# HaploConduct/HaploConduct

Hardware: AMD Instinct MI355X
Metric: candidate overlaps scored/sec (edge-calc scoring pass: compute_overlap + overlap_score + admission class, candidates resident in HBM; the whole stage from the overlaps text: stage_end_to_end) (higher is better)
Workload: dtype f64; 1 GPU; c3: 500000 synthetic 2x150 bp read pairs, 6 quality values (SURVEY 8(d)), 100000000 p-p candidates per GPU; read_pairs=500000, genome_len=90000, quality_alphabet=6, candidates_per_gpu=100000000, record_bytes=16, parallelism=candidate shards x1, replicated read store

## Files before the change

haploconduct_amd/csrc/hc_kernels.hip:

```cpp
#include <hip/hip_runtime.h>
#include <stdint.h>
#include <stdlib.h>

#include <algorithm>
#include <cstdio>
#include <string>

#include "../../include/hcedge.h"
#include "hc_device.h"
#include "hc_resolve.h"
#include "hc_ctx.h"

#ifndef HC_ABLATE
#define HC_ABLATE 0
#endif

namespace hc {

template <typename SymT, bool WIDE>
__global__ __launch_bounds__(256) void encode_store_kernel(const uint8_t* __restrict__ bases,
                                                           const uint8_t* __restrict__ quals,
                                                           const uint64_t* __restrict__ raw_off,
                                                           const uint64_t* __restrict__ seq_off,
                                                           const uint32_t* __restrict__ rc_delta,
                                                           const uint8_t* __restrict__ qmap,
                                                           uint32_t n_seq, uint32_t K, SymT* __restrict__ sym,
                                                           uint8_t* __restrict__ seq_bad, uint32_t slot_align) {
    const uint32_t lane = threadIdx.x & 63;
    const uint32_t wave = (blockIdx.x * blockDim.x + threadIdx.x) >> 6;
    const uint32_t n_waves = (gridDim.x * blockDim.x) >> 6;
    const bool dup = sizeof(SymT) == 1 && !WIDE && lut_lg(K) == 3;
    const SymT nsym = WIDE ? (SymT)(kWideN << 2) : (SymT)((K << 3) | kCodeN | (dup ? (K & 3u) << 6 : 0u));
    for (uint32_t q = wave; q < n_seq; q += n_waves) {
        const uint64_t r0 = raw_off[q];
        const uint32_t len = (uint32_t)(raw_off[q + 1] - r0);
        const uint64_t f0 = seq_off[q];
        const uint64_t stride = slot_stride(len, sizeof(SymT), slot_align);
        const uint64_t rc0 = f0 + rc_delta[q];
        uint32_t bad = 0;
        for (uint32_t i = lane; i < (uint32_t)stride; i += 64) {
            if (i < len) {
                const uint8_t b = bases[r0 + i];
                const uint8_t qi = qmap[quals[r0 + i]];
                uint32_t code;
                switch (b) {
                    case 'A': code = 0; break;
                    case 'C': code = 1; break;
                    case 'G': code = 2; break;
                    case 'T': code = 3; break;
                    case 'N': code = kCodeN; break;
                    default: code = kCodeBadBase; bad = 1; break;
                }
                uint32_t qx = qi;
                if (WIDE) {
                    uint32_t b2 = code < 4 ? code : 0u;
                    if (code == kCodeN) qx = kWideN;
                    if (code == kCodeBadBase) qx = kWideBadBase;
                    if (qi == 255) { qx = kWideBadQual; b2 = 0; }
                    const uint32_t rb2 = qx >= wide_first(lut_lg(K)) ? 3u - b2 : 0u;
                    sym[f0 + i] = (SymT)((qx << 2) | b2);
                    sym[rc0 + (len - 1 - i)] = (SymT)((qx << 2) | rb2);
                } else {
                    if (code == kCodeN) qx = K;
                    if (code == kCodeBadBase) qx = K + 1;
                    if (qi == 255) {
                        code = kCodeBadQual;
                        qx = K + 1;
                    }
                    const uint32_t rcode = code < 4 ? 3 - code : code;
                    const uint32_t qbits = (qx << 3) | (dup ? (qx & 3u) << 6 : 0u);
                    sym[f0 + i] = (SymT)(qbits | code);
                    sym[rc0 + (len - 1 - i)] = (SymT)(qbits | rcode);
                }
            } else {
                sym[f0 + i] = nsym;
                sym[rc0 + i] = nsym;
            }
        }
        const unsigned long long any_bad = __ballot(bad != 0);
        if (lane == 0) seq_bad[q] = any_bad ? 1 : 0;
    }
}

__global__ __launch_bounds__(256) void build_read_desc_kernel(const uint32_t* __restrict__ read_first_seq,
                                                              const uint64_t* __restrict__ seq_off,
                                                              const uint64_t* __restrict__ raw_off,
                                                              const uint8_t* __restrict__ seq_bad, const uint32_t* __restrict__ rc_delta,
                                                              uint32_t n_reads, ReadDesc* __restrict__ out) {
    const uint32_t r = blockIdx.x * blockDim.x + threadIdx.x;
    if (r >= n_reads) return;
    const uint32_t f = read_first_seq[r];
    const bool paired = (read_first_seq[r + 1] - f) == 2;
    ReadDesc d;
    d.off1 = seq_off[f];
    d.len1 = (uint32_t)(raw_off[f + 1] - raw_off[f]);
    d.flags = (paired ? kReadPaired : 0u) | (seq_bad[f] ? kReadBadBase1 : 0u);
    d.off2 = 0;
    d.len2 = 0;
    if (paired) {
        d.off2 = seq_off[f + 1];
        d.len2 = (uint32_t)(raw_off[f + 2] - raw_off[f + 1]);
        d.flags |= seq_bad[f + 1] ? kReadBadBase2 : 0u;
    }
    d.rc_delta = rc_delta[f];
    out[r] = d;
}

struct SubScore {
    double x;
    uint32_t mm, n;
    uint32_t err;
};

template <typename SymT>
struct Tr;
template <>
struct Tr<uint8_t> {
    static constexpr int kSymsPerWord = 4;
    static constexpr int kWords = 4;
    static constexpr uint32_t kLow1 = 0x01010101u;
    static constexpr int kSymBits = 8;
};
template <>
struct Tr<uint16_t> {
    static constexpr int kSymsPerWord = 2;
    static constexpr int kWords = 8;
    static constexpr uint32_t kLow1 = 0x00010001u;
    static constexpr int kSymBits = 16;
};

typedef const __attribute__((address_space(3))) double lds_cdouble;
__device__ __forceinline__ double lds_f64(uint32_t byte_addr) {
#if HC_ABLATE & 1
    return __hiloint2double(0x3C000000 | (int)(byte_addr & 0xFFFFu), (int)byte_addr);
#else
    return *(lds_cdouble*)(uintptr_t)byte_addr;
#endif
}

template <typename SymT>
__device__ __noinline__ SubScore score_sub_slow(const SymT* __restrict__ a, const SymT* __restrict__ b, uint32_t L, uint32_t Kp) {
    const uint32_t lg = lut_lg(Kp - 2u);
    SubScore r;
    r.x = -__builtin_inf();
    r.mm = 1;
    r.n = 1;
    r.err = 0;
    const bool wide = sizeof(SymT) == 1 && lg >= 6;
    auto kind = [&](uint32_t sy) -> uint32_t {
        if (wide) {
            const uint32_t q = sy >> 2;
            return q == kWideN ? 1u : (q == kWideBadQual ? 2u : (q == kWideBadBase ? 3u : 0u));
        }
        const uint32_t c = sy & 7u;
        return c == kCodeN ? 1u : (c == kCodeBadQual ? 2u : (c == kCodeBadBase ? 3u : 0u));
    };
    for (uint32_t i = 0; i < L; ++i)
        if (kind(a[i]) == 2u || kind(b[i]) == 2u) {
            r.err = 1;
            return r;
        }
    double S = 0.0;
    uint32_t cn = 0, cm = 0;
    for (uint32_t i = 0; i < L; ++i) {
        const uint32_t sa = a[i], sb = b[i];
        const uint32_t ka = kind(sa), kb = kind(sb);
        if (ka == 3u || kb == 3u) {
            r.err = 1;
            return r;
        }
        if (ka == 1u || kb == 1u) continue;
        const uint32_t m = wide ? ((sa & 3u) != (sb & 3u)) : ((sa & 7u) != (sb & 7u));
        const uint32_t qmask = sizeof(SymT) == 1 ? (1u << lg) - 1u : 0xFFFFu;
        const uint32_t qa = wide ? sa >> 2 : (sa >> 3) & qmask, qb = wide ? sb >> 2 : (sb >> 3) & qmask;
        const uint32_t addr = sizeof(SymT) == 1 ? lut_addr_u8(lg, qa, qb, m) : lut_addr_u16(Kp, qa, qb, m);
        const double t = lds_f64(addr);
        if (t == __builtin_inf()) return r;
        S += t;
        cn += 1;
        cm += m;
    }
    if (cn == 0) return r;
    r.x = (1.0 / (double)cn) * S;
    r.mm = cm;
    r.n = cn;
    return r;
}

template <typename SymT, int LG>
__device__ __forceinline__ void half_chunk_terms(const uint32_t* wa, const uint32_t* wb, uint32_t Kp, double (&t)[8], uint32_t& cn4,
                                                 uint32_t& cm4) {
    using T = Tr<SymT>;
#pragma unroll
    for (int jj = 0; jj < T::kWords / 2; ++jj) {
        const uint32_t aw = wa[jj];
        const uint32_t bw = wb[jj];
        const uint32_t e = aw ^ bw;
        if (sizeof(SymT) == 1 && LG >= 6) {
            constexpr uint32_t k80 = 0x80808080u;
            uint32_t ua = (aw << 1) | aw, ub = (bw << 1) | bw;
            if (LG == 7) {
                ua |= ua << 2;
                ub |= ub << 2;
            }
            const uint32_t nm = __builtin_amdgcn_bitop3_b32(ua, k80, ub, 0x4C);
            const uint32_t mk = __builtin_amdgcn_bitop3_b32((e << 7) | (e << 6), k80, nm, 0x40);
            asm("v_bcnt_u32_b32 %0, %1, %0" : "+v"(cn4) : "v"(nm));
            asm("v_bcnt_u32_b32 %0, %1, %0" : "+v"(cm4) : "v"(mk));
            const uint32_t lo = __builtin_amdgcn_bitop3_b32(e << 1, 0xF8F8F8F8u, aw, 0x48);
            const uint32_t z = __builtin_amdgcn_bitop3_b32(e >> 7, 0x01010101u, mk, 0xEA);
            const uint32_t hi = __builtin_amdgcn_bitop3_b32(aw >> 1, 0x7E7E7E7Eu, z, 0xE2);
#pragma unroll
            for (int k = 0; k < 4; ++k)
                t[jj * 4 + k] = lds_f64(__builtin_amdgcn_perm(hi, lo, 0x0C0C0000u | ((4u + k) << 8) | (uint32_t)k));
            continue;
        }
        constexpr uint32_t kFlag = T::kLow1 << 2;
        const uint32_t nm = __builtin_amdgcn_bitop3_b32(aw, kFlag, bw, 0xC8);
        const uint32_t mk = __builtin_amdgcn_bitop3_b32((e << 1) | (e << 2), kFlag, nm, 0x40);
        cn4 += nm;
        cm4 += mk;
        if (sizeof(SymT) == 1) {
            uint32_t lo, hi;
            if (LG == 5) {
                lo = e & 0xF8F8F8F8u;
                hi = ((aw >> 3) & 0x1F1F1F1Fu) | (mk << 3);
            } else if (LG == 4) {
                lo = (e & 0x78787878u) | ((aw << 4) & 0x80808080u);
                hi = ((aw >> 4) & 0x07070707u) | (mk << 1);
            } else {
                lo = (e & 0x38383838u) | (aw & 0xC0C0C0C0u);
                hi = (aw & 0x38383838u) | mk;
            }
#pragma unroll
            for (int k = 0; k < 4; ++k)
                t[jj * 4 + k] = lds_f64(__builtin_amdgcn_perm(hi, lo, 0x0C0C0000u | ((4u + k) << 8) | (uint32_t)k));
        } else {
            typedef unsigned short u16x2 __attribute__((ext_vector_type(2)));
            const u16x2 qa2 = __builtin_bit_cast(u16x2, aw) >> (unsigned short)3;
            const u16x2 qb2 = __builtin_bit_cast(u16x2, bw) >> (unsigned short)3;
            const u16x2 m2 = __builtin_bit_cast(u16x2, mk >> 2);
            const u16x2 hi2 = __builtin_elementwise_max(qa2, qb2), lo2 = __builtin_elementwise_min(qa2, qb2);
            const u16x2 one2 = {1, 1};
            const u16x2 tri2 = {(unsigned short)lut_tri(Kp), (unsigned short)lut_tri(Kp)};
            const uint32_t e2 = __builtin_bit_cast(uint32_t, (u16x2)(m2 * tri2 + (((hi2 * (hi2 + one2)) >> (unsigned short)1) + lo2)));
            t[jj * 2 + 0] = lds_f64((e2 << 3) & 0x7FFF8u);
            t[jj * 2 + 1] = lds_f64((e2 >> 13) & 0x7FFF8u);
        }
    }
}

template <typename SymT, int LG, int G >
__device__ __forceinline__ void score_sub_wide(const SymT* __restrict__ a, const SymT* __restrict__ b, uint32_t L, uint32_t fatal,
                                               uint32_t Kp, SubScore& out) {
    using T = Tr<SymT>;
    constexpr bool kPacked = !(sizeof(SymT) == 1 && LG >= 6);
    out.x = -__builtin_inf();
    out.mm = 1;
    out.n = 1;
    out.err = fatal;
    if (L == 0) return;
    const uint32_t nch = (L + 15u) >> 4;
    double S = 0.0;
    uint32_t skipped = 0, cm = 0;
    uint32_t xa[G][T::kWords], xb[G][T::kWords], ya[G][T::kWords], yb[G][T::kWords];
    auto fetch = [&](uint32_t (&ra)[G][T::kWords], uint32_t (&rb)[G][T::kWords], uint32_t cbase) {
#pragma unroll
        for (int q = 0; q < G; ++q)
            if (cbase + q < nch) {
                __builtin_memcpy(ra[q], a + 16u * (cbase + q), sizeof(ra[q]));
                __builtin_memcpy(rb[q], b + 16u * (cbase + q), sizeof(rb[q]));
            }
    };
    auto score_group = [&](const uint32_t (&ra)[G][T::kWords], const uint32_t (&rb)[G][T::kWords], uint32_t cbase) {
        uint32_t cn4 = 0, cm4 = 0;
#pragma unroll
        for (int q = 0; q < G; ++q)
            if (cbase + q < nch) {
#pragma unroll
                for (int h = 0; h < 2; ++h) {
                    double t[8];
                    half_chunk_terms<SymT, LG>(ra[q] + h * (T::kWords / 2), rb[q] + h * (T::kWords / 2), Kp, t, cn4, cm4);
#pragma unroll
                    for (int k = 0; k < 8; ++k) S += t[k];
                }
            }
        if (kPacked) {
            skipped = __builtin_amdgcn_sad_u8(cn4, 0u, skipped);
            cm = __builtin_amdgcn_sad_u8(cm4, 0u, cm);
        } else {
            skipped += cn4;
            cm += cm4;
        }
    };
    auto arrived = [](uint32_t (&rb)[G][T::kWords]) { asm volatile("" : "+v"(rb[G - 1][T::kWords - 1])); };
    fetch(xa, xb, 0);
    for (uint32_t c0 = 0; c0 < nch; c0 += 2 * G) {
        arrived(xb);
        fetch(ya, yb, c0 + G);
        score_group(xa, xb, c0);
        arrived(yb);
        fetch(xa, xb, c0 + 2 * G);
        score_group(ya, yb, c0 + G);
    }
    if (kPacked) {
        skipped >>= 2;
        cm >>= 2;
    }
    if (S != S) {
        const SubScore e = score_sub_slow<SymT>(a, b, L, Kp);
        out.x = e.x;
        out.mm = e.mm;
        out.n = e.n;
        out.err |= e.err;
        return;
    }
    if (S == __builtin_inf()) return;
    const uint32_t cn = 16u * nch - skipped;
    if (cn == 0) return;
    out.x = (1.0 / (double)cn) * S;
    out.mm = cm;
    out.n = cn;
}

typedef uint32_t u32x4 __attribute__((ext_vector_type(4)));
typedef __attribute__((address_space(3))) u32x4 lds_u32x4;
__device__ __forceinline__ void lds_store128(uint32_t addr, u32x4 v) { *(lds_u32x4*)(uintptr_t)addr = v; }
__device__ __forceinline__ u32x4 lds_load128(uint32_t addr) { return *(const lds_u32x4*)(uintptr_t)addr; }
typedef __attribute__((address_space(3))) uint32_t lds_u32;
typedef uint32_t u32x2 __attribute__((ext_vector_type(2)));
typedef __attribute__((address_space(3))) u32x2 lds_u32x2;
__device__ __forceinline__ void lds_store64(uint32_t addr, uint32_t a, uint32_t b) { *(lds_u32x2*)(uintptr_t)addr = u32x2{a, b}; }
__device__ __forceinline__ void lds_load64(uint32_t addr, uint32_t& a, uint32_t& b) {
    const u32x2 v = *(const lds_u32x2*)(uintptr_t)addr;
    a = v[0];
    b = v[1];
}
__device__ __forceinline__ uint32_t lds_load32(uint32_t addr) { return *(const lds_u32*)(uintptr_t)addr; }
__device__ __forceinline__ uint32_t lds_add_rtn(uint32_t addr, uint32_t v) {
    return __hip_atomic_fetch_add((lds_u32*)(uintptr_t)addr, v, __ATOMIC_RELAXED, __HIP_MEMORY_SCOPE_WORKGROUP);
}
__device__ __forceinline__ void wave_lds_order() {
    __builtin_amdgcn_fence(__ATOMIC_RELEASE, "wavefront");
    __builtin_amdgcn_wave_barrier();
}

constexpr uint32_t kStageBytesPerWave = 64u * 64u;
constexpr uint32_t kWideDmaLanes = 768, kWideDmaScratch = 3u << 9;
__host__ __device__ inline uint32_t coop_stage_base(uint32_t lut_bytes, uint32_t wg) {
    return (lut_bytes == 65536u && wg == kWideDmaLanes) ? 65536u : (lut_bytes + 128u + 1023u) & ~1023u;
}

template <typename SymT>
__device__ __forceinline__ void finish_sub(const SymT* __restrict__ sym, uint32_t offA, uint32_t offB, uint32_t L, uint32_t fatal, uint32_t Kp, double S,
                                           uint32_t skipped, uint32_t cm, bool packed, const double* __restrict__ inv_n, SubScore& out) {
    out.x = -__builtin_inf();
    out.mm = 1;
    out.n = 1;
    out.err = fatal;
    if (L == 0) return;
    if (packed) {
        skipped >>= 2;
        cm >>= 2;
    }
    if (S != S) {
        const SubScore e = score_sub_slow<SymT>((const SymT*)((const char*)sym + offA), (const SymT*)((const char*)sym + offB), L, Kp);
        out.x = e.x;
        out.mm = e.mm;
        out.n = e.n;
        out.err |= e.err;
        return;
    }
    if (S == __builtin_inf()) return;
    const uint32_t cn = 16u * ((L + 15u) >> 4) - skipped;
    if (cn == 0) return;
    out.x = inv_n[cn] * S;
    out.mm = cm;
    out.n = cn;
}

template <typename SymT, int LG, int DEPTH = 1>
__device__ __forceinline__ void score_sub_coop(__amdgpu_buffer_rsrc_t rsrc, uint32_t oob, const SymT* __restrict__ sym, uint32_t stage, uint32_t offA,
                                               uint32_t offB, uint32_t L, uint32_t fatal, uint32_t Kp, const double* __restrict__ inv_n, SubScore& out) {
    using T = Tr<SymT>;
    constexpr uint32_t kSymB = sizeof(SymT);
    constexpr int kChunks = 4 / kSymB;
    constexpr uint32_t kChunkB = 16u * kSymB;
    constexpr bool kPacked = !(sizeof(SymT) == 1 && LG >= 6);
    const uint32_t lane = threadIdx.x & 63u;
    const uint32_t piece = (lane & 3u) ^ ((lane >> 4) & 3u);
    const uint32_t Lb = L * kSymB;
    uint32_t la[4], lb[4], lim[4];
#pragma unroll
    for (int j = 0; j < 4; ++j) {
        const int src = 16 * j + (int)(lane >> 2);
        la[j] = (uint32_t)__shfl((int)offA, src, 64) + 16u * piece;
        lb[j] = (uint32_t)__shfl((int)offB, src, 64) + 16u * piece;
        const uint32_t end = (uint32_t)__shfl((int)Lb, src, 64), cs = (16u * piece) & ~(kChunkB - 1u);
        lim[j] = end > cs ? end - cs : 0u;
    }
    const uint32_t wr = stage + lane * 16u;
    const uint32_t rd = stage + lane * 64u + (((lane >> 2) & 3u) << 4);
    if constexpr (DEPTH == 0) {
        double S = 0.0;
        uint32_t skipped = 0, cm = 0;
        const uint32_t rdA = stage + lane * 64u + (((lane >> 2) & 3u) << 4), rdB = rdA + 4096u;
        auto fetch_dma = [&](uint32_t at) {
#pragma unroll
            for (int j = 0; j < 4; ++j) {
                const bool on = at < lim[j];
#if !(HC_ABLATE & 8)
                __builtin_amdgcn_raw_ptr_buffer_load_lds(rsrc, (__attribute__((address_space(3))) void*)(uintptr_t)(stage + 1024u * j), 16,
                                                         on ? la[j] : oob, at, 0, 0);
#endif
                __builtin_amdgcn_raw_ptr_buffer_load_lds(rsrc, (__attribute__((address_space(3))) void*)(uintptr_t)(stage + 4096u + 1024u * j), 16,
                                                         on ? lb[j] : oob, at, 0, 0);
            }
        };
#if HC_ABLATE & 16
        if (__ballot(Lb != 0u) != 0ull) {
            auto fetch_b = [&](uint32_t at, uint32_t half) {
#pragma unroll
                for (int j = 0; j < 4; ++j) {
                    const bool on = at < lim[j];
                    __builtin_amdgcn_raw_ptr_buffer_load_lds(rsrc, (__attribute__((address_space(3))) void*)(uintptr_t)(stage + 4096u * half + 1024u * j), 16,
                                                             on ? lb[j] : oob, at, 0, 0);
                }
            };
            fetch_b(0, 0);
            fetch_b(64u, 1);
            uint32_t half = 0;
            for (uint32_t at = 0;; at += 64u, half ^= 1u) {
                asm volatile("s_waitcnt vmcnt(4)" ::: "memory");
                wave_lds_order();
                u32x4 xa[4], xb[4];
                const uint32_t rdH = rdA + 4096u * half;
#pragma unroll
                for (int p = 0; p < 4; ++p) {
                    xb[p] = lds_load128(rdH ^ ((uint32_t)p << 4));
                    xa[p] = xb[p];
                }
                asm volatile("s_waitcnt lgkmcnt(0)" : "+v"(xa[0]), "+v"(xa[1]), "+v"(xa[2]), "+v"(xa[3]), "+v"(xb[0]), "+v"(xb[1]), "+v"(xb[2]), "+v"(xb[3])::"memory");
                wave_lds_order();
                const bool more = __ballot(at + 64u < Lb) != 0ull;
                fetch_b(at + 128u, half);
                uint32_t cn4 = 0, cm4 = 0;
#pragma unroll
                for (int q = 0; q < kChunks; ++q)
                    if (at + kChunkB * q < Lb) {
                        uint32_t wa[T::kWords], wb[T::kWords];
#pragma unroll
                        for (int sw = 0; sw < (int)kSymB; ++sw) {
                            const int p = q * (int)kSymB + sw;
#pragma unroll
                            for (int w = 0; w < 4; ++w) {
                                wa[4 * sw + w] = xa[p][w] ^ 0x08080808u;
                                wb[4 * sw + w] = xb[p][w];
                            }
                        }
#pragma unroll
                        for (int h = 0; h < 2; ++h) {
                            double t[8];
                            half_chunk_terms<SymT, LG>(wa + h * (T::kWords / 2), wb + h * (T::kWords / 2), Kp, t, cn4, cm4);
#pragma unroll
                            for (int k = 0; k < 8; ++k) S += t[k];
                        }
                    }
                skipped = __builtin_amdgcn_sad_u8(cn4, 0u, skipped);
                cm = __builtin_amdgcn_sad_u8(cm4, 0u, cm);
                if (!more) break;
            }
            asm volatile("s_waitcnt vmcnt(0)" ::: "memory");
        }
        finish_sub<SymT>(sym, offA, offB, L, fatal, Kp, S == S ? S : 0.0, skipped, cm, kPacked, inv_n, out);
        return;
#endif
        if (__ballot(Lb != 0u) != 0ull) {
            fetch_dma(0);
            for (uint32_t at = 0;; at += 64u) {
                asm volatile("s_waitcnt vmcnt(0)" ::: "memory");
                wave_lds_order();
                u32x4 xa[4], xb[4];
#pragma unroll
                for (int p = 0; p < 4; ++p) {
                    xb[p] = lds_load128(rdB ^ ((uint32_t)p << 4));
#if HC_ABLATE & 8
                    xa[p] = xb[p] ^ 0x08080808u;
#else
                    xa[p] = lds_load128(rdA ^ ((uint32_t)p << 4));
#endif
                }
                asm volatile("s_waitcnt lgkmcnt(0)" : "+v"(xa[0]), "+v"(xa[1]), "+v"(xa[2]), "+v"(xa[3]), "+v"(xb[0]), "+v"(xb[1]), "+v"(xb[2]), "+v"(xb[3])::"memory");
                wave_lds_order();
                const bool more = __ballot(at + 64u < Lb) != 0ull;
                if (more) fetch_dma(at + 64u);
                uint32_t cn4 = 0, cm4 = 0;
#pragma unroll
                for (int q = 0; q < kChunks; ++q)
                    if (at + kChunkB * q < Lb) {
                        uint32_t wa[T::kWords], wb[T::kWords];
#pragma unroll
                        for (int sw = 0; sw < (int)kSymB; ++sw) {
                            const int p = q * (int)kSymB + sw;
#pragma unroll
                            for (int w = 0; w < 4; ++w) {
                                wa[4 * sw + w] = xa[p][w];
                                wb[4 * sw + w] = xb[p][w];
                            }
                        }
#pragma unroll
                        for (int h = 0; h < 2; ++h) {
                            double t[8];
                            half_chunk_terms<SymT, LG>(wa + h * (T::kWords / 2), wb + h * (T::kWords / 2), Kp, t, cn4, cm4);
#pragma unroll
                            for (int k = 0; k < 8; ++k) S += t[k];
                        }
                    }
                if (kPacked) {
                    skipped = __builtin_amdgcn_sad_u8(cn4, 0u, skipped);
                    cm = __builtin_amdgcn_sad_u8(cm4, 0u, cm);
                } else {
                    skipped += cn4;
                    cm += cm4;
                }
                if (!more) break;
            }
        }
        finish_sub<SymT>(sym, offA, offB, L, fatal, Kp, S, skipped, cm, kPacked, inv_n, out);
        return;
    }
    u32x4 nA[DEPTH == 0 ? 1 : DEPTH][4], nB[DEPTH == 0 ? 1 : DEPTH][4];
    auto fetch = [&](u32x4 (&sA)[4], u32x4 (&sB)[4], uint32_t at) {
#pragma unroll
        for (int j = 0; j < 4; ++j) {
            const bool on = at < lim[j];
#if HC_ABLATE & 2
            sA[j] = u32x4{0x01010101u + (on ? (la[j] + at) & 0x02020202u : 0u), 0x01010101u, 0x09090909u, 0x11111111u};
            sB[j] = u32x4{0x09090909u + (on ? (lb[j] + at) & 0x02020202u : 0u), 0x09090909u, 0x01010101u, 0x11111111u};
#else
            sA[j] = __builtin_amdgcn_raw_buffer_load_b128(rsrc, on ? la[j] : oob, at, 0);
            sB[j] = __builtin_amdgcn_raw_buffer_load_b128(rsrc, on ? lb[j] : oob, at, 0);
#endif
        }
    };
    double S = 0.0;
    uint32_t skipped = 0, cm = 0;
    auto step = [&](u32x4 (&sA)[4], u32x4 (&sB)[4], uint32_t at) {
        u32x4 xa[4];
#if HC_ABLATE & 4
        u32x4 xb_[4];
#pragma unroll
        for (int p = 0; p < 4; ++p) {
            xa[p] = sA[p];
            xb_[p] = sB[p];
        }
#else
#pragma unroll
        for (int j = 0; j < 4; ++j) lds_store128(wr + 1024u * j, sA[j]);
        wave_lds_order();
#pragma unroll
        for (int p = 0; p < 4; ++p) xa[p] = lds_load128(rd ^ ((uint32_t)p << 4));
        wave_lds_order();
#pragma unroll
        for (int j = 0; j < 4; ++j) lds_store128(wr + 1024u * j, sB[j]);
        wave_lds_order();
#endif
        fetch(sA, sB, at + 64u * DEPTH);
        uint32_t cn4 = 0, cm4 = 0;
#pragma unroll
        for (int q = 0; q < kChunks; ++q)
            if (at + kChunkB * q < Lb) {
                uint32_t wa[T::kWords], wb[T::kWords];
#pragma unroll
                for (int s = 0; s < (int)kSymB; ++s) {
                    const int p = q * (int)kSymB + s;
#if HC_ABLATE & 4
                    const u32x4 vb = xb_[p];
#else
                    const u32x4 vb = lds_load128(rd ^ ((uint32_t)p << 4));
#endif
#pragma unroll
                    for (int w = 0; w < 4; ++w) {
                        wa[4 * s + w] = xa[p][w];
                        wb[4 * s + w] = vb[w];
                    }
                }
#pragma unroll
                for (int h = 0; h < 2; ++h) {
                    double t[8];
                    half_chunk_terms<SymT, LG>(wa + h * (T::kWords / 2), wb + h * (T::kWords / 2), Kp, t, cn4, cm4);
#pragma unroll
                    for (int k = 0; k < 8; ++k) S += t[k];
                }
            }
        if (kPacked) {
            skipped = __builtin_amdgcn_sad_u8(cn4, 0u, skipped);
            cm = __builtin_amdgcn_sad_u8(cm4, 0u, cm);
        } else {
            skipped += cn4;
            cm += cm4;
        }
        wave_lds_order();
    };
#pragma unroll
    for (int d = 0; d < DEPTH; ++d) fetch(nA[d], nB[d], 64u * d);
    for (uint32_t at = 0; __ballot(at < Lb) != 0ull; at += 64u * DEPTH) {
        step(nA[0], nB[0], at);
        if (DEPTH == 2) {
            if (__ballot(at + 64u < Lb) == 0ull) break;
            step(nA[DEPTH - 1], nB[DEPTH - 1], at + 64u);
        }
    }
    finish_sub<SymT>(sym, offA, offB, L, fatal, Kp, S, skipped, cm, kPacked, inv_n, out);
}

template <bool STREAM = true>
__device__ __forceinline__ void store_result(hc_result_rec* __restrict__ out, uint64_t i, const hc_result_rec& r) {
    unsigned long long* p = (unsigned long long*)(out + i);
    if (STREAM) {
        __builtin_nontemporal_store((unsigned long long)__double_as_longlong(r.x1), p);
        __builtin_nontemporal_store((unsigned long long)__double_as_longlong(r.x2), p + 1);
        __builtin_nontemporal_store(((unsigned long long)r.n_cls << 32) | r.mm, p + 2);
    } else {
        p[0] = (unsigned long long)__double_as_longlong(r.x1);
        p[1] = (unsigned long long)__double_as_longlong(r.x2);
        p[2] = ((unsigned long long)r.n_cls << 32) | r.mm;
    }
}

__device__ __forceinline__ uint32_t band_test(double x, const Band& b) { return x > b.hi ? 1u : (x <= b.lo ? 0u : 2u); }

template <bool STREAM = true>
__device__ __forceinline__ hc_result_rec classify_and_store(const ScoreParams& prm, int ns, const SubScore& s1, const SubScore& s2,
                                                            uint64_t i, hc_result_rec* __restrict__ out) {
    hc_result_rec res;
    uint32_t mm = s1.mm, nn = s1.n;
    if (ns == 2) {
        bool second;
        if ((s1.mm | s2.mm) < (1u << 24) && (s1.n | s2.n) < (1u << 26)) second = (uint64_t)s1.mm * s2.n < (uint64_t)s2.mm * s1.n;
        else second = (double)(float)s1.mm / (double)s1.n < (double)(float)s2.mm / (double)s2.n;
        if (second) {
            mm = s2.mm;
            nn = s2.n;
        }
    }
    const bool e_all = prm.flags & 1u, o_all = prm.flags & 2u;
    uint32_t e = e_all ? 1u : band_test(s1.x, prm.edge);
    uint32_t o = o_all ? 1u : band_test(s1.x, prm.ov);
    if (ns == 2) {
        const uint32_t e2 = e_all ? 1u : band_test(s2.x, prm.edge), o2 = o_all ? 1u : band_test(s2.x, prm.ov);
        e = (e == 0 || e2 == 0) ? 0u : ((e == 1 && e2 == 1) ? 1u : 2u);
        o = (o == 0 || o2 == 0) ? 0u : ((o == 1 && o2 == 1) ? 1u : 2u);
    }
    uint32_t cls;
    if (s1.err | s2.err) cls = HC_CLS_ERROR;
    else if (e == 1) cls = HC_CLS_EDGE;
    else if (e == 2) cls = HC_CLS_AMBIG;
    else if (prm.merge_contigs == 0.0 ? mm == 0u : (double)(float)mm / (double)nn <= prm.merge_contigs) cls = HC_CLS_EDGE_MC;
    else if (o == 1) cls = HC_CLS_NONEDGE;
    else if (o == 2) cls = HC_CLS_AMBIG;
    else cls = HC_CLS_DROP;
    res.x1 = s1.x;
    res.x2 = s2.x;
    res.mm = mm;
    res.n_cls = (nn & 0x0FFFFFFFu) | (cls << 28);
    store_result<STREAM>(out, i, res);
    return res;
}

template <typename SymT, int G, int LG>
__device__ __forceinline__ hc_result_rec score_candidate(const ScoreParams& prm, const SymT* __restrict__ sym, uint32_t Kp, int ns,
                                                         const Sub& sub0, const Sub& sub1, uint64_t i,
                                                         hc_result_rec* __restrict__ out) {
    if (ns <= 0) {
        hc_result_rec res;
        res.x1 = -__builtin_inf();
        res.x2 = __builtin_nan("");
        res.mm = 1;
        res.n_cls = 1u | ((ns == 0 ? HC_CLS_ERROR : HC_CLS_DROP) << 28);
        store_result(out, i, res);
        return res;
    }
    SubScore s1, s2;
    s2.x = __builtin_nan("");
    s2.mm = 0;
    s2.n = 1;
    s2.err = 0;
    const SymT* a1 = sym + sub1.offA + sub1.pos;
    const SymT* b1 = sym + sub1.offB;
    const uint32_t L1 = ns == 2 ? sub_positions(sub1, prm.min_read_len) | (sub1.fatal << 31) : 0u;
    score_sub_wide<SymT, LG, G>(sym + sub0.offA + sub0.pos, sym + sub0.offB, sub_positions(sub0, prm.min_read_len), sub0.fatal, Kp, s1);
    if (ns == 2) score_sub_wide<SymT, LG, G>(a1, b1, L1 & 0x7FFFFFFFu, L1 >> 31, Kp, s2);
    return classify_and_store(prm, ns, s1, s2, i, out);
}

struct RowSink {
    hc_gather_row* rows;
    unsigned long long* count;
    uint64_t cap;
    uint64_t base_index;
    const hc_line_rec* lines_in;
    hc_line_rec* lines_out;
    hc_gather_row* seg_buf;
    uint32_t* seg_count;
    uint32_t seg_rows;
    uint32_t spill_cap;
    hc_gather_row* spill_buf;
    uint32_t* spill_count;
    unsigned long long* started;
};

__device__ __forceinline__ void append_rows_block(const RowSink& sink, bool valid, const hc_result_rec& res, uint64_t i, uint32_t* lds4) {
    const bool keep = valid && (res.n_cls >> 28) != HC_CLS_DROP;
    const uint64_t m = __ballot(keep);
    const uint32_t lane = threadIdx.x & 63u, wave = threadIdx.x >> 6, n_waves = blockDim.x >> 6;
    if (lane == 0) lds4[wave] = (uint32_t)__popcll(m);
    __syncthreads();
    if (threadIdx.x == 0) {
        uint32_t total = 0;
        for (uint32_t w = 0; w < n_waves; w++) {
            const uint32_t c = lds4[w];
            lds4[w] = total;
            total += c;
        }
        unsigned long long base = 0;
        if (total) base = atomicAdd(sink.count, (unsigned long long)total);
        lds4[16] = (uint32_t)base;
        lds4[17] = (uint32_t)(base >> 32);
    }
    __syncthreads();
    if (keep) {
        const uint64_t base = ((uint64_t)lds4[17] << 32) | lds4[16];
        const uint64_t pos = base + lds4[wave] + (uint64_t)__popcll(m & ((1ull << lane) - 1ull));
        if (pos < sink.cap) {
            hc_gather_row r;
            r.index = sink.base_index + i;
            r.x1 = res.x1;
            r.x2 = res.x2;
            r.mm = res.mm;
            r.n_cls = res.n_cls;
            sink.rows[pos] = r;
            if (sink.lines_in) {
                const uint4* a = (const uint4*)(sink.lines_in + i);
                uint4* b = (uint4*)(sink.lines_out + pos);
                b[0] = a[0];
                b[1] = a[1];
                b[2] = a[2];
            }
        }
    }
    __syncthreads();
}

template <typename SymT, int LG>
__device__ __forceinline__ void load_log_table(double* lut_s, const double* __restrict__ lut_g, uint32_t lut_n, uint32_t tid, uint32_t n_threads) {
    if (sizeof(SymT) == 1 && LG == 3) {
        for (uint32_t e = tid; e < 128u; e += n_threads) {
            const uint32_t at = lut_addr_u8(3, e >> 4, (e >> 1) & 7u, e & 1u) >> 3;
            lut_s[at] = lut_g[at];
        }
    } else {
        for (uint32_t i = tid; i < lut_n; i += n_threads) lut_s[i] = lut_g[i];
    }
}

constexpr int kBalItems = 1;
template <typename SymT>
__device__ __forceinline__ void balanced_slots(const StoreView& st, const ScoreParams& prm, const void* __restrict__ in, uint64_t n,
                                               const uint32_t* __restrict__ perm, uint32_t fmt, uint64_t block_base, uint32_t* bal,
                                               uint64_t (&slots)[kBalItems]) {
    const uint32_t tid = threadIdx.x, W = blockDim.x;
    const uint32_t red = 128u + kBalItems * W;
    uint32_t chunks[kBalItems];
    uint32_t wmax = 0, wsum = 0;
#pragma unroll
    for (int k = 0; k < kBalItems; ++k) {
        const uint64_t slot = block_base + (uint64_t)k * W + tid;
        slots[k] = slot;
        uint32_t c = 0;
        if (slot < n) {
            const Cand rec = load_cand(in, perm ? (uint64_t)perm[slot] : slot, fmt);
            Sub s0, s1;
            const int ns = resolve<(int)sizeof(SymT)>(st, rec, s0, s1);
            if (ns >= 1) c = (sub_positions(s0, prm.min_read_len) + 15u) >> 4;
            if (ns == 2) c += (sub_positions(s1, prm.min_read_len) + 15u) >> 4;
        }
        chunks[k] = c;
        wmax = c > wmax ? c : wmax;
        wsum += c;
    }
#pragma unroll
    for (int o = 32; o > 0; o >>= 1) {
        const uint32_t m = (uint32_t)__shfl_xor((int)wmax, o, 64);
        wmax = m > wmax ? m : wmax;
        wsum += (uint32_t)__shfl_xor((int)wsum, o, 64);
    }
    if ((tid & 63u) == 0) {
        bal[red + (tid >> 6)] = wmax;
        bal[red + 16 + (tid >> 6)] = wsum;
    }
    if (tid < 128) bal[tid] = 0;
    __syncthreads();
    uint32_t bmax = 0, bsum = 0;
    for (uint32_t w = 0; w < (W >> 6); ++w) {
        bmax = bal[red + w] > bmax ? bal[red + w] : bmax;
        bsum += bal[red + 16 + w];
    }
    if (bmax >= 16u && (uint64_t)bmax * kBalItems * W > 2ull * bsum) {
        uint32_t cls[kBalItems];
#pragma unroll
        for (int k = 0; k < kBalItems; ++k) {
            uint32_t c = 0;
            if (chunks[k] > 1) {
                const uint32_t lg = 31u - (uint32_t)__builtin_clz(chunks[k]);
                c = lg * 4u + (lg >= 2 ? (chunks[k] >> (lg - 2)) & 3u : 0u);
            }
            cls[k] = c > 127u ? 127u : c;
            atomicAdd(&bal[cls[k]], 1u);
        }
        __syncthreads();
        if (tid < 64) {
            const uint32_t c0 = bal[127 - 2 * tid], c1 = bal[126 - 2 * tid];
            uint32_t incl = c0 + c1;
#pragma unroll
            for (int o = 1; o < 64; o <<= 1) {
                const uint32_t up = (uint32_t)__shfl_up((int)incl, o, 64);
                if ((int)tid >= o) incl += up;
            }
            const uint32_t excl = incl - (c0 + c1);
            bal[127 - 2 * tid] = excl;
            bal[126 - 2 * tid] = excl + c0;
        }
        __syncthreads();
#pragma unroll
        for (int k = 0; k < kBalItems; ++k) bal[128 + atomicAdd(&bal[cls[k]], 1u)] = (uint32_t)k * W + tid;
        __syncthreads();
#pragma unroll
        for (int k = 0; k < kBalItems; ++k) {
            const uint32_t rank = (k & 1) ? (uint32_t)(k + 1) * W - 1u - tid : (uint32_t)k * W + tid;
            slots[k] = block_base + bal[128 + rank];
        }
    }
    __syncthreads();
}

template <typename SymT, int G, int LG, bool BAL>
__device__ __forceinline__ void score_kernel_body(const StoreView& st, const ScoreParams& prm, const double* __restrict__ lut_g,
                                                  const void* __restrict__ in, uint64_t n, hc_result_rec* __restrict__ out,
                                                  const uint32_t* __restrict__ perm, const RowSink& sink) {
    if (prm.n_dev) {
        const uint64_t nd = *prm.n_dev;
        n = nd < n ? nd : n;
    }
    extern __shared__ __attribute__((aligned(16))) double lut_s[];
    if ((uint32_t)(uintptr_t)(__attribute__((address_space(3))) void*)lut_s != 0u) __builtin_trap();
    const uint32_t lut_n = st.lut_bytes >> 3;
    load_log_table<SymT, LG>(lut_s, lut_g, lut_n, threadIdx.x, blockDim.x);
    __syncthreads();

    const SymT* sym = (const SymT*)st.sym;
    const uint32_t Kp = st.K + 2u;
    const uint32_t fmt = prm.rec_fmt;
    uint32_t* bal = (uint32_t*)(lut_s + lut_n);
    const uint32_t tid = threadIdx.x;
    const uint64_t stride = (uint64_t)gridDim.x * blockDim.x;
    constexpr int kItems = BAL ? kBalItems : 1;
    for (uint64_t block_base = (uint64_t)blockIdx.x * blockDim.x * kItems; block_base < n; block_base += stride * kItems) {
        uint64_t slots[kBalItems];
        slots[0] = block_base + tid;
        if (BAL) balanced_slots<SymT>(st, prm, in, n, perm, fmt, block_base, bal, slots);
#pragma unroll 1
        for (int k = 0; k < kItems; ++k) {
            const uint64_t slot = slots[k];
            hc_result_rec res;
            res.n_cls = 0;
            uint64_t i = 0;
            if (slot < n) {
                i = perm ? (uint64_t)perm[slot] : slot;
                const Cand rec = load_cand(in, i, fmt);
                Sub sub0{}, sub1{};
                const int ns = resolve<(int)sizeof(SymT)>(st, rec, sub0, sub1);
                res = score_candidate<SymT, G, LG>(prm, sym, Kp, ns, sub0, sub1, i, out);
            }
            if (sink.rows) append_rows_block(sink, slot < n, res, i, bal);
        }
    }
}

__device__ __forceinline__ void append_rows_wave(const RowSink& sink, bool valid, const hc_result_rec& res, uint64_t i) {
    const bool keep = valid && (res.n_cls >> 28) != HC_CLS_DROP;
    const uint64_t m = __ballot(keep);
    if (m == 0ull) return;
    const uint32_t lane = threadIdx.x & 63u;
    unsigned long long base = 0;
    if (lane == 0) base = atomicAdd(sink.count, (unsigned long long)__popcll(m));
    base = __shfl(base, 0, 64);
    if (keep) {
        const uint64_t pos = base + (uint64_t)__popcll(m & ((1ull << lane) - 1ull));
        if (pos < sink.cap) {
            hc_gather_row r;
            r.index = sink.base_index + i;
            r.x1 = res.x1;
            r.x2 = res.x2;
            r.mm = res.mm;
            r.n_cls = res.n_cls;
            sink.rows[pos] = r;
            if (sink.lines_in) {
                const uint4* a = (const uint4*)(sink.lines_in + i);
                uint4* b = (uint4*)(sink.lines_out + pos);
                b[0] = a[0];
                b[1] = a[1];
                b[2] = a[2];
            }
        }
    }
}

__device__ __forceinline__ void append_rows_segment(const RowSink& sink, bool valid, const hc_result_rec& res, uint64_t i, uint32_t lds_counter) {
    const bool keep = valid && (res.n_cls >> 28) != HC_CLS_DROP;
    const uint64_t m = __ballot(keep);
    if (m == 0ull) return;
    const uint32_t lane = threadIdx.x & 63u;
    uint32_t base = 0;
    if (lane == 0) base = lds_add_rtn(lds_counter, (uint32_t)__popcll(m));
    base = (uint32_t)__shfl((int)base, 0, 64);
    if (keep) {
        const uint32_t pos = base + (uint32_t)__popcll(m & ((1ull << lane) - 1ull));
        if (pos < sink.seg_rows) {
            hc_gather_row r;
            r.index = sink.base_index + i;
            r.x1 = res.x1;
            r.x2 = res.x2;
            r.mm = res.mm;
            r.n_cls = res.n_cls;
            sink.seg_buf[(uint64_t)blockIdx.x * sink.seg_rows + pos] = r;
        }
    }
    if (base + (uint32_t)__popcll(m) > sink.seg_rows) {
        const bool over = keep && base + (uint32_t)__popcll(m & ((1ull << lane) - 1ull)) >= sink.seg_rows;
        const uint64_t mo = __ballot(over);
        uint32_t sbase = 0;
        if (lane == 0) sbase = atomicAdd(sink.spill_count, (uint32_t)__popcll(mo));
        sbase = (uint32_t)__shfl((int)sbase, 0, 64);
        if (over) {
            const uint32_t pos = sbase + (uint32_t)__popcll(mo & ((1ull << lane) - 1ull));
            if (pos < sink.spill_cap) {
                hc_gather_row r;
                r.index = sink.base_index + i;
                r.x1 = res.x1;
                r.x2 = res.x2;
                r.mm = res.mm;
                r.n_cls = res.n_cls;
                sink.spill_buf[pos] = r;
            }
        }
    }
}

__global__ __launch_bounds__(256) void sink_compact_kernel(const hc_gather_row* __restrict__ seg_buf, const uint32_t* __restrict__ seg_count, uint32_t seg_rows,
                                                           uint32_t G, hc_gather_row* __restrict__ rows, unsigned long long cap,
                                                           unsigned long long* __restrict__ count, const hc_gather_row* __restrict__ spill_buf,
                                                           const uint32_t* __restrict__ spill_count, uint32_t spill_cap, uint32_t* __restrict__ spill_next) {
    __shared__ unsigned long long part[8];
    const uint32_t g = blockIdx.x, tid = threadIdx.x;
    unsigned long long before = 0, all = 0;
    for (uint32_t k = tid; k < G; k += 256) {
        const uint32_t c = seg_count[k] < seg_rows ? seg_count[k] : seg_rows;
        if (k < g) before += c;
        all += c;
    }
    for (int o = 32; o > 0; o >>= 1) {
        before += __shfl_down(before, o, 64);
        all += __shfl_down(all, o, 64);
    }
    if ((tid & 63u) == 0) {
        part[tid >> 6] = before;
        part[4 + (tid >> 6)] = all;
    }
    __syncthreads();
    before = part[0] + part[1] + part[2] + part[3];
    all = part[4] + part[5] + part[6] + part[7];
    const uint32_t mine = seg_count[g] < seg_rows ? seg_count[g] : seg_rows;
    const uint4* src = (const uint4*)(seg_buf + (uint64_t)g * seg_rows);
    uint4* dst = (uint4*)(rows + before);
    const unsigned long long room = before < cap ? cap - before : 0ull;
    const uint32_t n_copy = mine < room ? mine : (uint32_t)room;
    for (uint32_t k = tid; k < 2u * n_copy; k += 256) dst[k] = src[k];
    const uint32_t spilled = *spill_count;
    if (spilled) {
        const uint32_t have = spilled < spill_cap ? spilled : spill_cap;
        for (uint64_t k = (uint64_t)g * 256 + tid; k < have; k += (uint64_t)G * 256) {
            if (all + k < cap) {
                ((uint4*)(rows + all + k))[0] = ((const uint4*)(spill_buf + k))[0];
                ((uint4*)(rows + all + k))[1] = ((const uint4*)(spill_buf + k))[1];
            }
        }
    }
    if (g == G - 1 && tid == 0) {
        count[0] = all + spilled;
        count[1] = 0;
        count[2] = 0;
        count[3] = 0;
        *spill_next = 0;
    }
}

__device__ __forceinline__ uint32_t length_class(uint32_t chunks) {
    if (chunks < 16u) return chunks;
    const uint32_t lg = 31u - (uint32_t)__builtin_clz(chunks);
    const uint32_t c = 16u + (lg - 4u) * 4u + ((chunks >> (lg - 2u)) & 3u);
    return c > 127u ? 127u : c;
}

constexpr uint32_t kBucketTile = 4096;
template <int SB>
__global__ __launch_bounds__(1024) void bucket_perm_kernel(StoreView st, uint32_t min_read_len, uint32_t fmt, const void* __restrict__ in, uint64_t n,
                                                           const unsigned long long* __restrict__ n_dev, const uint32_t* __restrict__ perm_in,
                                                           uint32_t* __restrict__ perm_out, uint32_t* __restrict__ queue) {
    if (n_dev) {
        const uint64_t nd = *n_dev;
        n = nd < n ? nd : n;
    }
    __shared__ uint32_t hist[129];
    const uint32_t tid = threadIdx.x;
    if (blockIdx.x == 0 && tid == 0) *queue = 0;
    if (tid < 129) hist[tid] = 0;
    __syncthreads();
    const uint64_t tile_base = (uint64_t)blockIdx.x * kBucketTile;
    uint32_t cls[4], idx[4];
#pragma unroll
    for (int k = 0; k < 4; ++k) {
        const uint64_t slot = tile_base + (uint32_t)k * 1024u + tid;
        cls[k] = 0;
        idx[k] = 0;
        if (slot < n) {
            idx[k] = perm_in ? perm_in[slot] : (uint32_t)slot;
            const Cand rec = load_cand(in, idx[k], fmt);
            Sub s0, s1;
            const int ns = resolve<SB>(st, rec, s0, s1);
            uint32_t c = 0;
            if (ns >= 1) c = (sub_positions(s0, min_read_len) + 15u) >> 4;
            if (ns == 2) c += (sub_positions(s1, min_read_len) + 15u) >> 4;
            cls[k] = length_class(c) + 1u;
        }
        atomicAdd(&hist[cls[k]], 1u);
    }
    __syncthreads();
    if (tid < 64) {
        const uint32_t hi = 128u - 2u * tid, lo = hi - 1u;
        const uint32_t c0 = hist[hi], c1 = hist[lo];
        uint32_t incl = c0 + c1;
#pragma unroll
        for (int o = 1; o < 64; o <<= 1) {
            const uint32_t up = (uint32_t)__shfl_up((int)incl, o, 64);
            if ((int)tid >= o) incl += up;
        }
        const uint32_t excl = incl - (c0 + c1);
        hist[hi] = excl;
        hist[lo] = excl + c0;
        if (tid == 63) hist[0] = incl;
    }
    __syncthreads();
#pragma unroll
    for (int k = 0; k < 4; ++k) {
        const uint32_t rank = atomicAdd(&hist[cls[k]], 1u);
        if (cls[k]) perm_out[tile_base + rank] = idx[k];
    }
}

template <typename SymT, int LG, int WG, bool SORT, bool DYN, int DEPTH = 1, bool WQ = false>
__global__ __launch_bounds__(WG, DEPTH == 2 ? 2 : (WG == 256 ? 4 : (WG == 512 ? 2 : 1))) void score_kernel_coop(StoreView st, ScoreParams prm, const double* __restrict__ lut_g,
                                                            const void* __restrict__ in, uint64_t n, hc_result_rec* __restrict__ out,
                                                            const uint32_t* __restrict__ perm, RowSink sink, uint32_t* __restrict__ queue) {
    static_assert(SORT && (WQ || !DYN), "score_kernel_coop: no launch takes the unsorted form or the bucketed form without tickets");
    const uint64_t n_hint = n;
    if (prm.n_dev) {
        const uint64_t nd = *prm.n_dev;
        n = nd < n ? nd : n;
    }
    extern __shared__ __attribute__((aligned(16))) double lut_s[];
    if ((uint32_t)(uintptr_t)(__attribute__((address_space(3))) void*)lut_s != 0u) __builtin_trap();
    const uint32_t lut_n = st.lut_bytes >> 3;
    load_log_table<SymT, LG>(lut_s, lut_g, lut_n, threadIdx.x, WG);
    constexpr bool kScratchInTable = sizeof(SymT) == 1 && LG >= 6 && WG == (int)kWideDmaLanes;
    uint32_t* scratch = kScratchInTable ? (uint32_t*)((char*)lut_s + kWideDmaScratch) : (uint32_t*)(lut_s + lut_n);
    if (kScratchInTable) __syncthreads();
    const uint32_t seg_counter = (uint32_t)(uintptr_t)(__attribute__((address_space(3))) void*)(scratch + 24);
    if (threadIdx.x == 0) {
        scratch[24] = 0;
        scratch[29] = 0;
        if (sink.started) atomicAdd(sink.started, 1ull);
    }
    __syncthreads();
    const uint32_t stage_base = coop_stage_base(st.lut_bytes, WG);
    const uint32_t stage = (uint32_t)__builtin_amdgcn_readfirstlane(
        (int)(stage_base + (threadIdx.x >> 6) * (DEPTH == 0 ? 2u * kStageBytesPerWave : kStageBytesPerWave)));
    const SymT* sym = (const SymT*)st.sym;
    const uint32_t Kp = st.K + 2u;
    const uint32_t fmt = prm.rec_fmt;
    const __amdgpu_buffer_rsrc_t rsrc = __builtin_amdgcn_make_buffer_rsrc((void*)st.sym, 0, (uint32_t)st.store_bytes, 0x00020000);
    const uint32_t oob = (uint32_t)st.store_bytes;
    const uint32_t tid = threadIdx.x;
    const uint64_t stride = (uint64_t)gridDim.x * WG;
    const uint32_t n_tiles = DYN ? (uint32_t)((n_hint + kBucketTile - 1) / kBucketTile) : 0u;
    const uint32_t n_pieces = n_tiles * (kBucketTile / WG);
    const uint32_t wq_steps = WQ ? ((prm.pad >> 8) & 0xFu) : 0u;
    const uint32_t dq_pieces = (DYN && WQ && blockIdx.x < n_pieces) ? (n_pieces - blockIdx.x + gridDim.x - 1) / gridDim.x : 0u;
    const uint32_t wq_items = !WQ ? 0u : (DYN ? dq_pieces * (uint32_t)(WG / 64) : (uint32_t)((n + 64ull * wq_steps - 1) / (64ull * wq_steps)));
    const uint32_t wq_per = !WQ ? 0u : (DYN ? wq_items : (wq_items + gridDim.x - 1) / gridDim.x);
    uint32_t wq_first = DYN ? 0u : blockIdx.x * wq_per, wq_end = wq_first + wq_per < wq_items ? wq_first + wq_per : wq_items;
    uint32_t xq_base = 0, xq_stride = 0;
    if (WQ && !DYN && prm.order_off) {
        if (*prm.order_off) {
            perm = nullptr;
        } else if (wq_items) {
            const uint32_t G = gridDim.x, g = blockIdx.x & 7u, l = blockIdx.x >> 3, q = G >> 3, r = G & 7u;
            const uint32_t m = q + (g < r ? 1u : 0u);
            const uint32_t g_start = (g * q + (g < r ? g : r)) * wq_per;
            const uint32_t g_end = g_start + m * wq_per < wq_items ? g_start + m * wq_per : wq_items;
            wq_first = 0;
            wq_end = g_end > g_start + l ? (g_end - g_start - l + m - 1) / m : 0u;
            xq_base = g_start + l;
            xq_stride = m;
        }
    }
    uint32_t wq_item = 0, wq_next_raw = 0, wq_k = 0;
    auto wq_pull = [&]() -> uint32_t {
        uint32_t t = 0;
        if ((tid & 63u) == 0) t = lds_add_rtn(seg_counter + 20u, 1u);
        return t;
    };
    if (WQ) {
        wq_item = wq_first + (tid >> 6);
        if (wq_item < wq_end) wq_next_raw = wq_pull();
    }
    for (uint64_t block_base = (uint64_t)blockIdx.x * WG;; block_base += stride) {
        uint64_t slot;
        if (WQ) {
            if (wq_k == wq_steps) {
                wq_item = wq_first + (uint32_t)(WG / 64) + (uint32_t)__builtin_amdgcn_readfirstlane((int)wq_next_raw);
                wq_k = 0;
                if (wq_item < wq_end) wq_next_raw = wq_pull();
            }
            if (wq_item >= wq_end) break;
            if (DYN) {
                const uint32_t k = wq_item / (uint32_t)(WG / 64), w = wq_item - k * (uint32_t)(WG / 64);
                const uint32_t q = blockIdx.x + k * gridDim.x;
                const uint32_t piece = q / n_tiles, tile = q - piece * n_tiles;
                slot = (uint64_t)tile * kBucketTile + piece * WG + w * 64u + (tid & 63u);
            } else {
                const uint32_t item = xq_stride ? xq_base + xq_stride * wq_item : wq_item;
                slot = ((uint64_t)item * wq_steps + wq_k) * 64u + (tid & 63u);
            }
            ++wq_k;
        } else {
            if (block_base >= n) break;
            slot = block_base + tid;
        }
        uint64_t i = 0;
        int ns = -2;
        uint32_t a0 = 0, b0 = 0, l0 = 0, a1 = 0, b1 = 0, l1 = 0;
        if (slot < n) {
            i = perm ? (uint64_t)perm[slot] : slot;
            const Cand rec = load_cand(in, i, fmt);
            if (st.regular) {
                ns = resolve_regular32<(int)sizeof(SymT)>(st, prm.min_read_len, rec, a0, b0, l0, a1, b1, l1);
            } else {
                Sub sub0{}, sub1{};
                ns = resolve<(int)sizeof(SymT)>(st, rec, sub0, sub1);
                if (ns >= 1) {
                    a0 = (uint32_t)((sub0.offA + sub0.pos) * sizeof(SymT));
                    b0 = (uint32_t)(sub0.offB * sizeof(SymT));
                    l0 = sub_positions(sub0, prm.min_read_len) | (sub0.fatal << 31);
                }
                if (ns == 2) {
                    a1 = (uint32_t)((sub1.offA + sub1.pos) * sizeof(SymT));
                    b1 = (uint32_t)(sub1.offB * sizeof(SymT));
                    l1 = sub_positions(sub1, prm.min_read_len) | (sub1.fatal << 31);
                }
            }
        }
        const uint32_t L0 = l0 & 0x7FFFFFFFu, L1 = l1 & 0x7FFFFFFFu;
        SubScore s1, s2;
        {
            const uint32_t lane = tid & 63u;
            const uint32_t c0 = length_class((L0 + 15u) >> 4), c1 = length_class((L1 + 15u) >> 4);
            const uint32_t hb = stage + 2048u;
            lds_store64(hb + 8u * lane, 0u, 0u);
            wave_lds_order();
            const uint32_t bin0 = hb + 4u * (127u - c0), bin1 = hb + 4u * (127u - c1);
            uint32_t r0 = lds_add_rtn(bin0, 1u);
            uint32_t r1 = lds_add_rtn(bin1, 1u);
            wave_lds_order();
            {
                uint32_t h0, h1;
                lds_load64(hb + 8u * lane, h0, h1);
                uint32_t incl = h0 + h1;
#pragma unroll
                for (int o = 1; o < 64; o <<= 1) {
                    const uint32_t up = (uint32_t)__shfl_up((int)incl, o, 64);
                    if ((int)lane >= o) incl += up;
                }
                const uint32_t excl = incl - (h0 + h1);
                wave_lds_order();
                lds_store64(hb + 8u * lane, excl, excl + h0);
            }
            wave_lds_order();
            r0 += lds_load32(bin0);
            r1 += lds_load32(bin1);
            wave_lds_order();
            const uint32_t x = stage;
            lds_store128(x + 16u * r0, u32x4{a0, b0, l0, 2u * lane});
            lds_store128(x + 16u * r1, u32x4{a1, b1, l1, 2u * lane + 1u});
            wave_lds_order();
            const u32x4 p0 = lds_load128(x + 16u * lane), p1 = lds_load128(x + 16u * (127u - lane));
            wave_lds_order();
            SubScore r[2];
            score_sub_coop<SymT, LG, DEPTH>(rsrc, oob, sym, stage, p0[0], p0[1], p0[2] & 0x7FFFFFFFu, p0[2] >> 31, Kp, st.inv_n, r[0]);
            r[1].x = -__builtin_inf();
            r[1].mm = 1;
            r[1].n = 1;
            r[1].err = p1[2] >> 31;
            if (__ballot((p1[2] & 0x7FFFFFFFu) != 0u) != 0ull)
                score_sub_coop<SymT, LG, DEPTH>(rsrc, oob, sym, stage, p1[0], p1[1], p1[2] & 0x7FFFFFFFu, p1[2] >> 31, Kp, st.inv_n, r[1]);
            wave_lds_order();
            lds_store128(x + 16u * p0[3], u32x4{(uint32_t)__double2loint(r[0].x), (uint32_t)__double2hiint(r[0].x), r[0].mm, r[0].n | (r[0].err << 31)});
            lds_store128(x + 16u * p1[3], u32x4{(uint32_t)__double2loint(r[1].x), (uint32_t)__double2hiint(r[1].x), r[1].mm, r[1].n | (r[1].err << 31)});
            wave_lds_order();
            const u32x4 q0 = lds_load128(x + 32u * lane), q1 = lds_load128(x + 32u * lane + 16u);
            wave_lds_order();
            s1.x = __hiloint2double((int)q0[1], (int)q0[0]);
            s1.mm = q0[2];
            s1.n = q0[3] & 0x7FFFFFFFu;
            s1.err = q0[3] >> 31;
            s2.x = __hiloint2double((int)q1[1], (int)q1[0]);
            s2.mm = q1[2];
            s2.n = q1[3] & 0x7FFFFFFFu;
            s2.err = q1[3] >> 31;
        }
        if (ns != 2) {
            s2.x = __builtin_nan("");
            s2.mm = 0;
            s2.n = 1;
            s2.err = 0;
        }
        hc_result_rec res;
        res.n_cls = 0;
        if (slot < n) {
            if (ns <= 0) {
                res.x1 = -__builtin_inf();
                res.x2 = __builtin_nan("");
                res.mm = 1;
                res.n_cls = 1u | ((ns == 0 ? HC_CLS_ERROR : HC_CLS_DROP) << 28);
                store_result<!DYN>(out, i, res);
            } else {
                res = classify_and_store<!DYN>(prm, ns, s1, s2, i, out);
            }
        }
        if (sink.rows) {
            if (sink.seg_count) append_rows_segment(sink, slot < n, res, i, seg_counter);
            else if (DYN) append_rows_wave(sink, slot < n, res, i);
            else append_rows_block(sink, slot < n, res, i, scratch);
        }
    }
    if (sink.rows && sink.seg_count) {
        __syncthreads();
        if (threadIdx.x == 0) sink.seg_count[blockIdx.x] = scratch[24];
    }
}

template <typename SymT, int G, int LG, bool BAL>
__global__ __launch_bounds__(256, sizeof(SymT) == 1 ? 4 : 3) void score_kernel(StoreView st, ScoreParams prm, const double* __restrict__ lut_g,
                                                    const void* __restrict__ in, uint64_t n, hc_result_rec* __restrict__ out,
                                                    const uint32_t* __restrict__ perm, RowSink sink) {
    score_kernel_body<SymT, G, LG, BAL>(st, prm, lut_g, in, n, out, perm, sink);
}

template <typename SymT, int G, int LG>
__global__ __launch_bounds__(512, 4) void score_kernel_wide_wg(StoreView st, ScoreParams prm, const double* __restrict__ lut_g,
                                                            const void* __restrict__ in, uint64_t n,
                                                            hc_result_rec* __restrict__ out, const uint32_t* __restrict__ perm,
                                                            RowSink sink) {
    score_kernel_body<SymT, G, LG, false>(st, prm, lut_g, in, n, out, perm, sink);
}

hipError_t launch_encode(uint32_t symbytes, const uint8_t* bases, const uint8_t* quals, const uint64_t* raw_off,
                         const uint64_t* seq_off, const uint32_t* rc_delta, const uint8_t* qmap, uint32_t n_seq, uint32_t K, void* sym,
                         uint8_t* seq_bad, const uint32_t* read_first_seq, uint32_t n_reads, ReadDesc* descs, uint32_t slot_align,
                         hipStream_t stream) {
    if (n_seq == 0) return hipSuccess;
    const uint32_t waves_per_block = 4;
    uint32_t blocks = (n_seq + waves_per_block - 1) / waves_per_block;
    if (blocks > 65536) blocks = 65536;
    if (symbytes == 1 && lut_lg(K) >= 6)
        hipLaunchKernelGGL((encode_store_kernel<uint8_t, true>), dim3(blocks), dim3(256), 0, stream, bases, quals, raw_off,
                           seq_off, rc_delta, qmap, n_seq, K, (uint8_t*)sym, seq_bad, slot_align);
    else if (symbytes == 1)
        hipLaunchKernelGGL((encode_store_kernel<uint8_t, false>), dim3(blocks), dim3(256), 0, stream, bases, quals, raw_off,
                           seq_off, rc_delta, qmap, n_seq, K, (uint8_t*)sym, seq_bad, slot_align);
    else
        hipLaunchKernelGGL((encode_store_kernel<uint16_t, false>), dim3(blocks), dim3(256), 0, stream, bases, quals, raw_off,
                           seq_off, rc_delta, qmap, n_seq, K, (uint16_t*)sym, seq_bad, slot_align);
    hipError_t e = hipGetLastError();
    if (e != hipSuccess) return e;
    if (n_reads)
        hipLaunchKernelGGL(build_read_desc_kernel, dim3((n_reads + 255) / 256), dim3(256), 0, stream, read_first_seq,
                           seq_off, raw_off, seq_bad, rc_delta, n_reads, descs);
    return hipGetLastError();
}

#define HC_WQ_NAME_true ", true"
#define HC_WQ_NAME_false ""
#define HC_LANE(T, G, LG, BAL) \
    {false, sizeof(T), LG, 256, G, BAL, 0, false, (const void*)&score_kernel<T, G, LG, BAL>, "hc::score_kernel<" #T ", " #G ", " #LG ", " #BAL ">"}
#define HC_LANE2(T, G, LG) HC_LANE(T, G, LG, false), HC_LANE(T, G, LG, true)
#define HC_LANE512(G, LG) \
    {false, 1, LG, 512, G, false, 0, false, (const void*)&score_kernel_wide_wg<uint8_t, G, LG>, "hc::score_kernel_wide_wg<uint8_t, " #G ", " #LG ">"}
#define HC_COOP(T, LG, WG, DYN, DEPTH, WQ)                                                                                       \
    {true, sizeof(T), LG, WG, 0, DYN, DEPTH, WQ, (const void*)&score_kernel_coop<T, LG, WG, true, DYN, DEPTH, WQ>,              \
     "hc::score_kernel_coop<" #T ", " #LG ", " #WG ", true, " #DYN ", " #DEPTH HC_WQ_NAME_##WQ ">"}
#define HC_COOP1024(T, LG) HC_COOP(T, LG, 1024, false, 1, false), HC_COOP(T, LG, 1024, false, 1, true), HC_COOP(T, LG, 1024, true, 1, true)
static_assert(kWideDmaLanes == 768, "the table names the wide LDS-DMA form's workgroup size");
static const ScoreKernel kScoreKernels[] = {
    HC_LANE2(uint8_t, 4, 3), HC_LANE2(uint8_t, 2, 3), HC_LANE2(uint8_t, 4, 4), HC_LANE2(uint8_t, 2, 4), HC_LANE2(uint8_t, 4, 5), HC_LANE2(uint8_t, 2, 5),
    HC_LANE(uint8_t, 4, 6, true), HC_LANE(uint8_t, 2, 6, true), HC_LANE(uint8_t, 4, 7, true), HC_LANE(uint8_t, 2, 7, true),
    HC_LANE512(4, 6), HC_LANE512(2, 6), HC_LANE512(4, 7), HC_LANE512(2, 7), HC_LANE2(uint16_t, 2, 5),
    HC_COOP(uint8_t, 3, 256, false, 1, false), HC_COOP(uint8_t, 4, 256, false, 1, false), HC_COOP(uint8_t, 5, 256, false, 1, false),
    HC_COOP(uint8_t, 3, 256, true, 2, true), HC_COOP(uint8_t, 4, 256, true, 2, true), HC_COOP(uint8_t, 5, 256, true, 2, true),
    HC_COOP(uint8_t, 3, 1024, false, 0, false), HC_COOP(uint8_t, 4, 1024, false, 0, false), HC_COOP(uint8_t, 5, 1024, false, 0, false),
    HC_COOP(uint8_t, 3, 1024, false, 0, true), HC_COOP(uint8_t, 4, 1024, false, 0, true), HC_COOP(uint8_t, 5, 1024, false, 0, true),
    HC_COOP1024(uint8_t, 6), HC_COOP1024(uint8_t, 7), HC_COOP1024(uint16_t, 5),
    HC_COOP(uint8_t, 6, 768, false, 0, true), HC_COOP(uint8_t, 7, 768, false, 0, true),
};
#undef HC_WQ_NAME_true
#undef HC_WQ_NAME_false
#undef HC_LANE
#undef HC_LANE2
#undef HC_LANE512
#undef HC_COOP
#undef HC_COOP1024

static const ScoreKernel* find_score_kernel(const ScoreKernel& key) {
    for (const ScoreKernel& k : kScoreKernels)
        if (k.coop == key.coop && k.symbytes == key.symbytes && k.lg == key.lg && k.wg == key.wg && k.group == key.group && k.bal == key.bal &&
            k.depth == key.depth && k.wq == key.wq)
            return &k;
    return nullptr;
}

constexpr size_t kLdsBytes = 160 * 1024;
constexpr uint64_t kDmaMinCandidates = 150000;
constexpr uint32_t kTicketSteps = 1;
constexpr uint64_t kDmaGridPerCu = 16, kGridPerSlot = 4;
static uint64_t coop_dma_min() {
    const char* e = getenv("HC_COOP_DMA_MIN");
    return e ? strtoull(e, nullptr, 10) : kDmaMinCandidates;
}
static bool wide_dma_wanted() {
    const char* e = getenv("HC_WIDE_DMA");
    return !(e && atoi(e) == 0);
}

ScorePlan plan_score_launch(const StoreView& st, bool coop_fetch, int lane_group, uint32_t n_cu, uint64_t n, RowSinkKind sink) {
    ScorePlan p;
    const uint32_t lg = lut_lg(st.K), lgt = st.symbytes == 2 ? 5u : lg;
    ScoreKernel key{};
    key.symbytes = st.symbytes;
    key.lg = lgt;
    const size_t lds_256 = coop_stage_base(st.lut_bytes, 256) + 4 * kStageBytesPerWave;
    const uint32_t wg_c = 4 * lds_256 <= kLdsBytes ? 256u : 1024u;
    const size_t lds_c = coop_stage_base(st.lut_bytes, wg_c) + (wg_c / 64) * kStageBytesPerWave;
    if (coop_fetch && st.store_bytes < 0xFFFF0000ull && lds_c <= kLdsBytes) {
        uint32_t per_cu = std::min<uint32_t>((uint32_t)(kLdsBytes / lds_c), 32 / (wg_c / 64));
        p.lds = p.lds_form = lds_c;
        if ((st.long_rows || st.balance) && wg_c == 256 && per_cu > 2) {
            per_cu = 2;
            p.lds = std::max(lds_c, kLdsBytes / 3 + 1024);
        }
        p.waves_per_cu = per_cu * (wg_c / 64);
        p.bucketed = st.balance && n < (1ull << 32);
        const bool tickets_ok = sink != RowSinkKind::unsegmented;
        const bool tickets = p.bucketed || (wg_c == 1024 && tickets_ok);
        key.coop = true;
        key.wg = wg_c;
        key.bal = p.bucketed;
        key.depth = p.bucketed && per_cu <= 2 && wg_c == 256 ? 2 : 1;
        key.wq = tickets;
        p.kernel = p.staged = find_score_kernel(key);
        p.blocks = (uint32_t)std::min<uint64_t>((n + wg_c - 1) / wg_c, (uint64_t)n_cu * per_cu * (tickets ? 1 : kGridPerSlot));
        if (n >= coop_dma_min() && !p.bucketed && st.symbytes == 1) {
            const size_t lds_dma = coop_stage_base(st.lut_bytes, 1024) + 16 * 2 * kStageBytesPerWave;
            const bool wide = lg >= 6 && st.lut_bytes == 65536u && wide_dma_wanted() && tickets_ok;
            if (wide || (lg <= 5 && lds_dma <= kLdsBytes)) {
                key.wg = wide ? kWideDmaLanes : 1024u;
                key.bal = false;
                key.depth = 0;
                key.wq = tickets_ok;
                p.kernel = find_score_kernel(key);
                p.lds = p.lds_form = wide ? kLdsBytes : lds_dma;
                p.waves_per_cu = key.wg / 64;
                p.blocks = (uint32_t)std::min<uint64_t>((n + key.wg - 1) / key.wg, (uint64_t)n_cu * (tickets_ok ? 1 : kDmaGridPerCu));
            }
        }
        p.segmented = sink == RowSinkKind::segmented && p.blocks <= kSinkMaxGroups;
        return p;
    }
    auto lds_for = [&](uint32_t lanes) { return st.lut_bytes + (128 + (st.balance ? kBalItems : 1) * lanes + 32) * sizeof(uint32_t); };
    const uint32_t per_cu = std::max<uint32_t>(1, std::min<uint32_t>(8, (uint32_t)(kLdsBytes / lds_for(256))));
    key.wg = (!st.balance && st.symbytes == 1 && lg >= 6 && per_cu <= 2) ? 512u : 256u;
    key.group = st.symbytes == 2 || lane_group == 2 ? 2 : 4;
    key.bal = st.balance && key.wg == 256;
    p.kernel = find_score_kernel(key);
    p.lds = p.lds_form = lds_for(key.wg);
    const uint64_t per_wg = (uint64_t)key.wg * (st.balance ? kBalItems : 1);
    p.blocks = (uint32_t)std::min<uint64_t>((n + per_wg - 1) / per_wg, (uint64_t)n_cu * per_cu * kGridPerSlot);
    return p;
}

hipError_t launch_score(const ScorePlan& plan, const StoreView& st, ScoreParams prm, const double* lut_g, const void* in, uint64_t n,
                        hc_result_rec* out, const uint32_t* perm, const ScoreBuffers& b, hipStream_t stream, uint32_t* started_groups) {
    if (started_groups) *started_groups = 0;
    if (n == 0) return hipSuccess;
    if (!plan.kernel) return hipErrorInvalidConfiguration;
    const ScoreKernel& k = *plan.kernel;
    if (plan.bucketed) {
        const uint32_t tiles = (uint32_t)((n + kBucketTile - 1) / kBucketTile);
        if (st.symbytes == 2)
            hipLaunchKernelGGL((bucket_perm_kernel<2>), dim3(tiles), dim3(1024), 0, stream, st, prm.min_read_len, prm.rec_fmt, in, n, prm.n_dev, perm,
                               b.bucket_perm, b.bucket_queue);
        else
            hipLaunchKernelGGL((bucket_perm_kernel<1>), dim3(tiles), dim3(1024), 0, stream, st, prm.min_read_len, prm.rec_fmt, in, n, prm.n_dev, perm,
                               b.bucket_perm, b.bucket_queue);
        perm = b.bucket_perm;
    }
    RowSink sink{b.rows, b.row_count, b.cap, b.base_index, b.lines_in, b.lines_out, nullptr, nullptr, 0u, 0u, nullptr, nullptr, k.coop ? b.started : nullptr};
    const uint64_t spill_at = b.seg_total_rows - b.cap;
    if (plan.segmented) {
        sink.seg_buf = b.seg_buf;
        sink.seg_count = b.seg_count;
        sink.seg_rows = (uint32_t)std::min<uint64_t>(spill_at / plan.blocks, 0xFFFFFFFFull);
        sink.spill_buf = b.seg_buf + spill_at;
        sink.spill_cap = (uint32_t)b.cap;
        sink.spill_count = b.seg_count + kSinkMaxGroups + (*b.spill_turn & 1u);
    } else if (b.rows) {
        const hipError_t ze = hipMemsetAsync(b.row_count, 0, sizeof(hc_gather_row), stream);
        if (ze != hipSuccess) return ze;
    }
    if (k.wq) prm.pad = (prm.pad & 0xFFu) | (kTicketSteps << 8);
    uint32_t* queue = plan.bucketed ? b.bucket_queue : nullptr;
    void* args[] = {(void*)&st, &prm, &lut_g, &in, &n, &out, &perm, &sink, &queue};
    const hipError_t le = hipLaunchKernel(k.fn, dim3(plan.blocks), dim3(k.wg), args, plan.lds, stream);
    if (plan.segmented) {
        hipLaunchKernelGGL(sink_compact_kernel, dim3(plan.blocks), dim3(256), 0, stream, (const hc_gather_row*)b.seg_buf, (const uint32_t*)b.seg_count,
                           sink.seg_rows, plan.blocks, b.rows, (unsigned long long)b.cap, b.row_count, (const hc_gather_row*)sink.spill_buf,
                           (const uint32_t*)sink.spill_count, sink.spill_cap, b.seg_count + kSinkMaxGroups + ((*b.spill_turn + 1u) & 1u));
        ++*b.spill_turn;
    }
    if (started_groups && k.coop) *started_groups = plan.blocks;
    const hipError_t e = hipGetLastError();
    return le != hipSuccess ? le : e;
}

std::string describe_score_kernel(const StoreView& st, bool coop_fetch, int lane_group, uint32_t n_cu, uint64_t n) {
    const uint64_t dma_min = coop_dma_min();
    const ScorePlan p = plan_score_launch(st, coop_fetch, lane_group, n_cu, n ? n : std::max<uint64_t>(dma_min, 1), RowSinkKind::none);
    if (!p.kernel) return "no scoring kernel for this read set";
    const uint32_t lg = lut_lg(st.K);
    const char* enc = st.symbytes == 2 ? "u16" : (lg >= 6 ? "wide8" : "packed8");
    char buf[640];
    if (!p.kernel->coop)
        snprintf(buf, sizeof buf, "%s encoding=%s table_bytes=%u (one lane, one fetch)", p.kernel->name, enc, st.lut_bytes);
    else if (p.kernel->depth == 0)
        snprintf(buf, sizeof buf, "%s encoding=%s table_bytes=%u lds_bytes=%zu waves_per_cu=%u LDS-DMA fetch for launches of %llu candidates and more "
                                  "(one workgroup per CU, the waves take their items from a ticket counter in LDS%s); smaller launches: %s",
                 p.kernel->name, enc, st.lut_bytes, p.lds_form, p.waves_per_cu, (unsigned long long)dma_min,
                 p.kernel->wg == kWideDmaLanes ? "; the scratch words sit in an unaddressed row of the table" : "", p.staged->name);
    else
        snprintf(buf, sizeof buf, "%s encoding=%s table_bytes=%u lds_bytes=%zu waves_per_cu=%u%s", p.kernel->name, enc, st.lut_bytes, p.lds_form,
                 p.waves_per_cu, p.bucketed ? " length-bucketed (hc::bucket_perm_kernel, items by ticket)" : "");
    return buf;
}

hipError_t set_score_kernel_lds_limit() {
    for (const ScoreKernel& k : kScoreKernels) {
        const hipError_t e = hipFuncSetAttribute(k.fn, hipFuncAttributeMaxDynamicSharedMemorySize, (int)kLdsBytes);
        if (e != hipSuccess) return e;
    }
    return hipSuccess;
}

}
```

haploconduct_amd/csrc/hc_resolve.h:

```cpp
#pragma once
#include <hip/hip_runtime.h>
#include <stdint.h>

#include "../../include/hcedge.h"
#include "hc_device.h"

namespace hc {

struct Cand {
    uint32_t read1, read2, pos1, pos2;
    uint32_t ori1, ori2;
    uint32_t ord;
    uint32_t skip;
};

__device__ __forceinline__ Cand load_cand(const void* __restrict__ in, uint64_t i, uint32_t fmt) {
    Cand c;
    typedef uint32_t u32x4_t __attribute__((ext_vector_type(4)));
    if (fmt == HC_REC_COMPACT) {
        const u32x4_t a = __builtin_nontemporal_load((const u32x4_t*)in + i);
        c.read1 = a.x;
        c.read2 = a.y;
        c.pos1 = a.z & HC_CAND_POS_MASK;
        c.pos2 = a.w & HC_CAND_POS_MASK;
        c.skip = a.w & HC_CAND_SKIP;
        c.ori1 = (a.z >> 28) & 1u;
        c.ori2 = (a.z >> 29) & 1u;
        const uint32_t oc = a.z >> 30;
        c.ord = oc == 1u ? (uint32_t)'1' : (oc == 2u ? (uint32_t)'2' : (oc == 0u ? (uint32_t)'-' : 0u));
    } else {
        const u32x4_t a = __builtin_nontemporal_load((const u32x4_t*)in + 2 * i);
        c.read1 = a.x;
        c.read2 = a.y;
        c.pos1 = a.z;
        c.pos2 = a.w;
        const uint32_t w = ((const uint32_t*)in)[8 * i + 4];
        c.ori1 = (w & 0xFFu) ? 1u : 0u;
        c.ori2 = ((w >> 8) & 0xFFu) ? 1u : 0u;
        c.ord = (w >> 16) & 0xFFu;
        c.skip = 0;
    }
    return c;
}

struct View {
    uint64_t off;
    uint32_t len;
    uint32_t fatal;
};

__device__ __forceinline__ ReadDesc load_desc(const ReadDesc* p) {
    const uint4* q = (const uint4*)p;
    const uint4 a = q[0], b = q[1];
    ReadDesc d;
    d.off1 = ((uint64_t)a.y << 32) | a.x;
    d.off2 = ((uint64_t)a.w << 32) | a.z;
    d.len1 = b.x;
    d.len2 = b.y;
    d.flags = b.z;
    d.rc_delta = b.w;
    return d;
}

__device__ __forceinline__ ReadDesc regular_desc(const StoreView& st, uint32_t r) {
    const bool paired = r >= st.n_single;
    const uint32_t seq = paired ? st.n_single + 2u * (r - st.n_single) : r;
    ReadDesc d;
    const uint32_t slot = st.seq_syms >> 1;
    d.off1 = (uint64_t)seq * st.seq_syms;
    d.off2 = paired ? d.off1 + slot : 0u;
    d.len1 = st.ulen;
    d.len2 = paired ? st.ulen : 0u;
    d.flags = paired ? kReadPaired : 0u;
    d.rc_delta = paired ? 2u * slot : slot;
    return d;
}

template <int SB>
__device__ __forceinline__ View make_view(const ReadDesc& d, uint32_t mate, uint32_t fwd) {
    View v;
    const uint64_t off = mate ? d.off2 : d.off1;
    v.len = mate ? d.len2 : d.len1;
    v.off = off + (fwd ? 0u : d.rc_delta);
    v.fatal = (!fwd && (d.flags & (mate ? kReadBadBase2 : kReadBadBase1))) ? 1u : 0u;
    return v;
}

struct Sub {
    uint64_t offA, offB;
    uint32_t lenA, lenB, pos, fatal;
};

__device__ __forceinline__ Sub make_sub(const View& A, const View& B, uint32_t pos) {
    Sub s;
    s.offA = A.off;
    s.offB = B.off;
    s.lenA = A.len;
    s.lenB = B.len;
    s.pos = pos;
    s.fatal = A.fatal | B.fatal;
    return s;
}

template <int SB>
__device__ __forceinline__ int resolve(const StoreView& st, const Cand& r, Sub& s0, Sub& s1) {
    if (r.skip) return -1;
    if (r.read1 >= st.n_reads || r.read2 >= st.n_reads || r.read1 == r.read2) return 0;
    const ReadDesc d1 = st.regular ? regular_desc(st, r.read1) : load_desc(st.reads + r.read1);
    const ReadDesc d2 = st.regular ? regular_desc(st, r.read2) : load_desc(st.reads + r.read2);
    const uint32_t p1 = d1.flags & kReadPaired, p2 = d2.flags & kReadPaired;
    const uint32_t o1 = r.ori1, o2 = r.ori2;
    const View F1 = make_view<SB>(d1, p1 ? (o1 ? 0u : 1u) : 0u, o1);
    const View F2 = make_view<SB>(d2, p2 ? (o2 ? 0u : 1u) : 0u, o2);
    s0 = make_sub(F1, F2, r.pos1);
    if (!p1 && !p2) return 1;
    const View K1 = make_view<SB>(d1, p1 ? (o1 ? 1u : 0u) : 0u, o1);
    const View K2 = make_view<SB>(d2, p2 ? (o2 ? 1u : 0u) : 0u, o2);
    if (!p1) {
        s1 = make_sub(F1, K2, r.pos2);
    } else if (!p2) {
        s1 = make_sub(F2, K1, r.pos2);
    } else {
        if (r.ord == '1') s1 = make_sub(K1, K2, r.pos2);
        else if (r.ord == '2') s1 = make_sub(K2, K1, r.pos2);
        else return 0;
    }
    return 2;
}

template <int SB>
__device__ __forceinline__ int resolve_regular32(const StoreView& st, uint32_t min_read_len, const Cand& r, uint32_t& a0, uint32_t& b0, uint32_t& L0,
                                                 uint32_t& a1, uint32_t& b1, uint32_t& L1) {
    a0 = b0 = L0 = a1 = b1 = L1 = 0u;
    if (r.skip) return -1;
    if (r.read1 >= st.n_reads || r.read2 >= st.n_reads || r.read1 == r.read2) return 0;
    const uint32_t slot = st.seq_syms >> 1;
    const bool p1 = r.read1 >= st.n_single, p2 = r.read2 >= st.n_single;
    const uint32_t base1 = (p1 ? 2u * r.read1 - st.n_single : r.read1) * st.seq_syms;
    const uint32_t base2 = (p2 ? 2u * r.read2 - st.n_single : r.read2) * st.seq_syms;
    const uint32_t F1 = base1 + (r.ori1 ? 0u : (p1 ? 3u * slot : slot));
    const uint32_t F2 = base2 + (r.ori2 ? 0u : (p2 ? 3u * slot : slot));
    const uint32_t ok = st.ulen >= min_read_len ? st.ulen : 0u;
    a0 = (F1 + r.pos1) * SB;
    b0 = F2 * SB;
    L0 = r.pos1 < ok ? ok - r.pos1 : 0u;
    if (!p1 && !p2) return 1;
    const uint32_t K1 = p1 ? base1 + (r.ori1 ? slot : 2u * slot) : F1;
    const uint32_t K2 = p2 ? base2 + (r.ori2 ? slot : 2u * slot) : F2;
    uint32_t A, B;
    if (!p1) {
        A = F1;
        B = K2;
    } else if (!p2) {
        A = F2;
        B = K1;
    } else if (r.ord == '1') {
        A = K1;
        B = K2;
    } else if (r.ord == '2') {
        A = K2;
        B = K1;
    } else {
        return 0;
    }
    a1 = (A + r.pos2) * SB;
    b1 = B * SB;
    L1 = r.pos2 < ok ? ok - r.pos2 : 0u;
    return 2;
}

__device__ __forceinline__ uint32_t sub_positions(const Sub& s, uint32_t min_read_len) {
    if (s.pos >= s.lenA) return 0;
    if (s.lenA < min_read_len || s.lenB < min_read_len) return 0;
    const uint32_t rem = s.lenA - s.pos;
    return rem < s.lenB ? rem : s.lenB;
}

}
```

Baseline: 17.26 billion candidate overlaps/s.

## Read coop kernel args from kernarg segment and branchless resolve/finish

```diff
diff --git a/haploconduct_amd/csrc/hc_kernels.hip b/haploconduct_amd/csrc/hc_kernels.hip
--- a/haploconduct_amd/csrc/hc_kernels.hip
+++ b/haploconduct_amd/csrc/hc_kernels.hip
@@ -351,349 +351,6 @@
     return (lut_bytes == 65536u && wg == kWideDmaLanes) ? 65536u : (lut_bytes + 128u + 1023u) & ~1023u;
 }
 
-template <typename SymT>
-__device__ __forceinline__ void finish_sub(const SymT* __restrict__ sym, uint32_t offA, uint32_t offB, uint32_t L, uint32_t fatal, uint32_t Kp, double S,
-                                           uint32_t skipped, uint32_t cm, bool packed, const double* __restrict__ inv_n, SubScore& out) {
-    out.x = -__builtin_inf();
-    out.mm = 1;
-    out.n = 1;
-    out.err = fatal;
-    if (L == 0) return;
-    if (packed) {
-        skipped >>= 2;
-        cm >>= 2;
-    }
-    if (S != S) {
-        const SubScore e = score_sub_slow<SymT>((const SymT*)((const char*)sym + offA), (const SymT*)((const char*)sym + offB), L, Kp);
-        out.x = e.x;
-        out.mm = e.mm;
-        out.n = e.n;
-        out.err |= e.err;
-        return;
-    }
-    if (S == __builtin_inf()) return;
-    const uint32_t cn = 16u * ((L + 15u) >> 4) - skipped;
-    if (cn == 0) return;
-    out.x = inv_n[cn] * S;
-    out.mm = cm;
-    out.n = cn;
-}
-
-template <typename SymT, int LG, int DEPTH = 1>
-__device__ __forceinline__ void score_sub_coop(__amdgpu_buffer_rsrc_t rsrc, uint32_t oob, const SymT* __restrict__ sym, uint32_t stage, uint32_t offA,
-                                               uint32_t offB, uint32_t L, uint32_t fatal, uint32_t Kp, const double* __restrict__ inv_n, SubScore& out) {
-    using T = Tr<SymT>;
-    constexpr uint32_t kSymB = sizeof(SymT);
-    constexpr int kChunks = 4 / kSymB;
-    constexpr uint32_t kChunkB = 16u * kSymB;
-    constexpr bool kPacked = !(sizeof(SymT) == 1 && LG >= 6);
-    const uint32_t lane = threadIdx.x & 63u;
-    const uint32_t piece = (lane & 3u) ^ ((lane >> 4) & 3u);
-    const uint32_t Lb = L * kSymB;
-    uint32_t la[4], lb[4], lim[4];
-#pragma unroll
-    for (int j = 0; j < 4; ++j) {
-        const int src = 16 * j + (int)(lane >> 2);
-        la[j] = (uint32_t)__shfl((int)offA, src, 64) + 16u * piece;
-        lb[j] = (uint32_t)__shfl((int)offB, src, 64) + 16u * piece;
-        const uint32_t end = (uint32_t)__shfl((int)Lb, src, 64), cs = (16u * piece) & ~(kChunkB - 1u);
-        lim[j] = end > cs ? end - cs : 0u;
-    }
-    const uint32_t wr = stage + lane * 16u;
-    const uint32_t rd = stage + lane * 64u + (((lane >> 2) & 3u) << 4);
-    if constexpr (DEPTH == 0) {
-        double S = 0.0;
-        uint32_t skipped = 0, cm = 0;
-        const uint32_t rdA = stage + lane * 64u + (((lane >> 2) & 3u) << 4), rdB = rdA + 4096u;
-        auto fetch_dma = [&](uint32_t at) {
-#pragma unroll
-            for (int j = 0; j < 4; ++j) {
-                const bool on = at < lim[j];
-#if !(HC_ABLATE & 8)
-                __builtin_amdgcn_raw_ptr_buffer_load_lds(rsrc, (__attribute__((address_space(3))) void*)(uintptr_t)(stage + 1024u * j), 16,
-                                                         on ? la[j] : oob, at, 0, 0);
-#endif
-                __builtin_amdgcn_raw_ptr_buffer_load_lds(rsrc, (__attribute__((address_space(3))) void*)(uintptr_t)(stage + 4096u + 1024u * j), 16,
-                                                         on ? lb[j] : oob, at, 0, 0);
-            }
-        };
-#if HC_ABLATE & 16
-        if (__ballot(Lb != 0u) != 0ull) {
-            auto fetch_b = [&](uint32_t at, uint32_t half) {
-#pragma unroll
-                for (int j = 0; j < 4; ++j) {
-                    const bool on = at < lim[j];
-                    __builtin_amdgcn_raw_ptr_buffer_load_lds(rsrc, (__attribute__((address_space(3))) void*)(uintptr_t)(stage + 4096u * half + 1024u * j), 16,
-                                                             on ? lb[j] : oob, at, 0, 0);
-                }
-            };
-            fetch_b(0, 0);
-            fetch_b(64u, 1);
-            uint32_t half = 0;
-            for (uint32_t at = 0;; at += 64u, half ^= 1u) {
-                asm volatile("s_waitcnt vmcnt(4)" ::: "memory");
-                wave_lds_order();
-                u32x4 xa[4], xb[4];
-                const uint32_t rdH = rdA + 4096u * half;
-#pragma unroll
-                for (int p = 0; p < 4; ++p) {
-                    xb[p] = lds_load128(rdH ^ ((uint32_t)p << 4));
-                    xa[p] = xb[p];
-                }
-                asm volatile("s_waitcnt lgkmcnt(0)" : "+v"(xa[0]), "+v"(xa[1]), "+v"(xa[2]), "+v"(xa[3]), "+v"(xb[0]), "+v"(xb[1]), "+v"(xb[2]), "+v"(xb[3])::"memory");
-                wave_lds_order();
-                const bool more = __ballot(at + 64u < Lb) != 0ull;
-                fetch_b(at + 128u, half);
-                uint32_t cn4 = 0, cm4 = 0;
-#pragma unroll
-                for (int q = 0; q < kChunks; ++q)
-                    if (at + kChunkB * q < Lb) {
-                        uint32_t wa[T::kWords], wb[T::kWords];
-#pragma unroll
-                        for (int sw = 0; sw < (int)kSymB; ++sw) {
-                            const int p = q * (int)kSymB + sw;
-#pragma unroll
-                            for (int w = 0; w < 4; ++w) {
-                                wa[4 * sw + w] = xa[p][w] ^ 0x08080808u;
-                                wb[4 * sw + w] = xb[p][w];
-                            }
-                        }
-#pragma unroll
-                        for (int h = 0; h < 2; ++h) {
-                            double t[8];
-                            half_chunk_terms<SymT, LG>(wa + h * (T::kWords / 2), wb + h * (T::kWords / 2), Kp, t, cn4, cm4);
-#pragma unroll
-                            for (int k = 0; k < 8; ++k) S += t[k];
-                        }
-                    }
-                skipped = __builtin_amdgcn_sad_u8(cn4, 0u, skipped);
-                cm = __builtin_amdgcn_sad_u8(cm4, 0u, cm);
-                if (!more) break;
-            }
-            asm volatile("s_waitcnt vmcnt(0)" ::: "memory");
-        }
-        finish_sub<SymT>(sym, offA, offB, L, fatal, Kp, S == S ? S : 0.0, skipped, cm, kPacked, inv_n, out);
-        return;
-#endif
-        if (__ballot(Lb != 0u) != 0ull) {
-            fetch_dma(0);
-            for (uint32_t at = 0;; at += 64u) {
-                asm volatile("s_waitcnt vmcnt(0)" ::: "memory");
-                wave_lds_order();
-                u32x4 xa[4], xb[4];
-#pragma unroll
-                for (int p = 0; p < 4; ++p) {
-                    xb[p] = lds_load128(rdB ^ ((uint32_t)p << 4));
-#if HC_ABLATE & 8
-                    xa[p] = xb[p] ^ 0x08080808u;
-#else
-                    xa[p] = lds_load128(rdA ^ ((uint32_t)p << 4));
-#endif
-                }
-                asm volatile("s_waitcnt lgkmcnt(0)" : "+v"(xa[0]), "+v"(xa[1]), "+v"(xa[2]), "+v"(xa[3]), "+v"(xb[0]), "+v"(xb[1]), "+v"(xb[2]), "+v"(xb[3])::"memory");
-                wave_lds_order();
-                const bool more = __ballot(at + 64u < Lb) != 0ull;
-                if (more) fetch_dma(at + 64u);
-                uint32_t cn4 = 0, cm4 = 0;
-#pragma unroll
-                for (int q = 0; q < kChunks; ++q)
-                    if (at + kChunkB * q < Lb) {
-                        uint32_t wa[T::kWords], wb[T::kWords];
-#pragma unroll
-                        for (int sw = 0; sw < (int)kSymB; ++sw) {
-                            const int p = q * (int)kSymB + sw;
-#pragma unroll
-                            for (int w = 0; w < 4; ++w) {
-                                wa[4 * sw + w] = xa[p][w];
-                                wb[4 * sw + w] = xb[p][w];
-                            }
-                        }
-#pragma unroll
-                        for (int h = 0; h < 2; ++h) {
-                            double t[8];
-                            half_chunk_terms<SymT, LG>(wa + h * (T::kWords / 2), wb + h * (T::kWords / 2), Kp, t, cn4, cm4);
-#pragma unroll
-                            for (int k = 0; k < 8; ++k) S += t[k];
-                        }
-                    }
-                if (kPacked) {
-                    skipped = __builtin_amdgcn_sad_u8(cn4, 0u, skipped);
-                    cm = __builtin_amdgcn_sad_u8(cm4, 0u, cm);
-                } else {
-                    skipped += cn4;
-                    cm += cm4;
-                }
-                if (!more) break;
-            }
-        }
-        finish_sub<SymT>(sym, offA, offB, L, fatal, Kp, S, skipped, cm, kPacked, inv_n, out);
-        return;
-    }
-    u32x4 nA[DEPTH == 0 ? 1 : DEPTH][4], nB[DEPTH == 0 ? 1 : DEPTH][4];
-    auto fetch = [&](u32x4 (&sA)[4], u32x4 (&sB)[4], uint32_t at) {
-#pragma unroll
-        for (int j = 0; j < 4; ++j) {
-            const bool on = at < lim[j];
-#if HC_ABLATE & 2
-            sA[j] = u32x4{0x01010101u + (on ? (la[j] + at) & 0x02020202u : 0u), 0x01010101u, 0x09090909u, 0x11111111u};
-            sB[j] = u32x4{0x09090909u + (on ? (lb[j] + at) & 0x02020202u : 0u), 0x09090909u, 0x01010101u, 0x11111111u};
-#else
-            sA[j] = __builtin_amdgcn_raw_buffer_load_b128(rsrc, on ? la[j] : oob, at, 0);
-            sB[j] = __builtin_amdgcn_raw_buffer_load_b128(rsrc, on ? lb[j] : oob, at, 0);
-#endif
-        }
-    };
-    double S = 0.0;
-    uint32_t skipped = 0, cm = 0;
-    auto step = [&](u32x4 (&sA)[4], u32x4 (&sB)[4], uint32_t at) {
-        u32x4 xa[4];
-#if HC_ABLATE & 4
-        u32x4 xb_[4];
-#pragma unroll
-        for (int p = 0; p < 4; ++p) {
-            xa[p] = sA[p];
-            xb_[p] = sB[p];
-        }
-#else
-#pragma unroll
-        for (int j = 0; j < 4; ++j) lds_store128(wr + 1024u * j, sA[j]);
-        wave_lds_order();
-#pragma unroll
-        for (int p = 0; p < 4; ++p) xa[p] = lds_load128(rd ^ ((uint32_t)p << 4));
-        wave_lds_order();
-#pragma unroll
-        for (int j = 0; j < 4; ++j) lds_store128(wr + 1024u * j, sB[j]);
-        wave_lds_order();
-#endif
-        fetch(sA, sB, at + 64u * DEPTH);
-        uint32_t cn4 = 0, cm4 = 0;
-#pragma unroll
-        for (int q = 0; q < kChunks; ++q)
-            if (at + kChunkB * q < Lb) {
-                uint32_t wa[T::kWords], wb[T::kWords];
-#pragma unroll
-                for (int s = 0; s < (int)kSymB; ++s) {
-                    const int p = q * (int)kSymB + s;
-#if HC_ABLATE & 4
-                    const u32x4 vb = xb_[p];
-#else
-                    const u32x4 vb = lds_load128(rd ^ ((uint32_t)p << 4));
-#endif
-#pragma unroll
-                    for (int w = 0; w < 4; ++w) {
-                        wa[4 * s + w] = xa[p][w];
-                        wb[4 * s + w] = vb[w];
-                    }
-                }
-#pragma unroll
-                for (int h = 0; h < 2; ++h) {
-                    double t[8];
-                    half_chunk_terms<SymT, LG>(wa + h * (T::kWords / 2), wb + h * (T::kWords / 2), Kp, t, cn4, cm4);
-#pragma unroll
-                    for (int k = 0; k < 8; ++k) S += t[k];
-                }
-            }
-        if (kPacked) {
-            skipped = __builtin_amdgcn_sad_u8(cn4, 0u, skipped);
-            cm = __builtin_amdgcn_sad_u8(cm4, 0u, cm);
-        } else {
-            skipped += cn4;
-            cm += cm4;
-        }
-        wave_lds_order();
-    };
-#pragma unroll
-    for (int d = 0; d < DEPTH; ++d) fetch(nA[d], nB[d], 64u * d);
-    for (uint32_t at = 0; __ballot(at < Lb) != 0ull; at += 64u * DEPTH) {
-        step(nA[0], nB[0], at);
-        if (DEPTH == 2) {
-            if (__ballot(at + 64u < Lb) == 0ull) break;
-            step(nA[DEPTH - 1], nB[DEPTH - 1], at + 64u);
-        }
-    }
-    finish_sub<SymT>(sym, offA, offB, L, fatal, Kp, S, skipped, cm, kPacked, inv_n, out);
-}
-
-template <bool STREAM = true>
-__device__ __forceinline__ void store_result(hc_result_rec* __restrict__ out, uint64_t i, const hc_result_rec& r) {
-    unsigned long long* p = (unsigned long long*)(out + i);
-    if (STREAM) {
-        __builtin_nontemporal_store((unsigned long long)__double_as_longlong(r.x1), p);
-        __builtin_nontemporal_store((unsigned long long)__double_as_longlong(r.x2), p + 1);
-        __builtin_nontemporal_store(((unsigned long long)r.n_cls << 32) | r.mm, p + 2);
-    } else {
-        p[0] = (unsigned long long)__double_as_longlong(r.x1);
-        p[1] = (unsigned long long)__double_as_longlong(r.x2);
-        p[2] = ((unsigned long long)r.n_cls << 32) | r.mm;
-    }
-}
-
-__device__ __forceinline__ uint32_t band_test(double x, const Band& b) { return x > b.hi ? 1u : (x <= b.lo ? 0u : 2u); }
-
-template <bool STREAM = true>
-__device__ __forceinline__ hc_result_rec classify_and_store(const ScoreParams& prm, int ns, const SubScore& s1, const SubScore& s2,
-                                                            uint64_t i, hc_result_rec* __restrict__ out) {
-    hc_result_rec res;
-    uint32_t mm = s1.mm, nn = s1.n;
-    if (ns == 2) {
-        bool second;
-        if ((s1.mm | s2.mm) < (1u << 24) && (s1.n | s2.n) < (1u << 26)) second = (uint64_t)s1.mm * s2.n < (uint64_t)s2.mm * s1.n;
-        else second = (double)(float)s1.mm / (double)s1.n < (double)(float)s2.mm / (double)s2.n;
-        if (second) {
-            mm = s2.mm;
-            nn = s2.n;
-        }
-    }
-    const bool e_all = prm.flags & 1u, o_all = prm.flags & 2u;
-    uint32_t e = e_all ? 1u : band_test(s1.x, prm.edge);
-    uint32_t o = o_all ? 1u : band_test(s1.x, prm.ov);
-    if (ns == 2) {
-        const uint32_t e2 = e_all ? 1u : band_test(s2.x, prm.edge), o2 = o_all ? 1u : band_test(s2.x, prm.ov);
-        e = (e == 0 || e2 == 0) ? 0u : ((e == 1 && e2 == 1) ? 1u : 2u);
-        o = (o == 0 || o2 == 0) ? 0u : ((o == 1 && o2 == 1) ? 1u : 2u);
-    }
-    uint32_t cls;
-    if (s1.err | s2.err) cls = HC_CLS_ERROR;
-    else if (e == 1) cls = HC_CLS_EDGE;
-    else if (e == 2) cls = HC_CLS_AMBIG;
-    else if (prm.merge_contigs == 0.0 ? mm == 0u : (double)(float)mm / (double)nn <= prm.merge_contigs) cls = HC_CLS_EDGE_MC;
-    else if (o == 1) cls = HC_CLS_NONEDGE;
-    else if (o == 2) cls = HC_CLS_AMBIG;
-    else cls = HC_CLS_DROP;
-    res.x1 = s1.x;
-    res.x2 = s2.x;
-    res.mm = mm;
-    res.n_cls = (nn & 0x0FFFFFFFu) | (cls << 28);
-    store_result<STREAM>(out, i, res);
-    return res;
-}
-
-template <typename SymT, int G, int LG>
-__device__ __forceinline__ hc_result_rec score_candidate(const ScoreParams& prm, const SymT* __restrict__ sym, uint32_t Kp, int ns,
-                                                         const Sub& sub0, const Sub& sub1, uint64_t i,
-                                                         hc_result_rec* __restrict__ out) {
-    if (ns <= 0) {
-        hc_result_rec res;
-        res.x1 = -__builtin_inf();
-        res.x2 = __builtin_nan("");
-        res.mm = 1;
-        res.n_cls = 1u | ((ns == 0 ? HC_CLS_ERROR : HC_CLS_DROP) << 28);
-        store_result(out, i, res);
-        return res;
-    }
-    SubScore s1, s2;
-    s2.x = __builtin_nan("");
-    s2.mm = 0;
-    s2.n = 1;
-    s2.err = 0;
-    const SymT* a1 = sym + sub1.offA + sub1.pos;
-    const SymT* b1 = sym + sub1.offB;
-    const uint32_t L1 = ns == 2 ? sub_positions(sub1, prm.min_read_len) | (sub1.fatal << 31) : 0u;
-    score_sub_wide<SymT, LG, G>(sym + sub0.offA + sub0.pos, sym + sub0.offB, sub_positions(sub0, prm.min_read_len), sub0.fatal, Kp, s1);
-    if (ns == 2) score_sub_wide<SymT, LG, G>(a1, b1, L1 & 0x7FFFFFFFu, L1 >> 31, Kp, s2);
-    return classify_and_store(prm, ns, s1, s2, i, out);
-}
-
 struct RowSink {
     hc_gather_row* rows;
     unsigned long long* count;
@@ -709,6 +366,376 @@
     uint32_t* spill_count;
     unsigned long long* started;
 };
+
+struct CoopArgs {
+    StoreView st;
+    ScoreParams prm;
+    const double* lut_g;
+    const void* in;
+    uint64_t n;
+    hc_result_rec* out;
+    const uint32_t* perm;
+    RowSink sink;
+    uint32_t* queue;
+};
+typedef const __attribute__((address_space(4))) CoopArgs* coop_args_ptr;
+__device__ __forceinline__ coop_args_ptr coop_args_here() {
+    coop_args_ptr p = (coop_args_ptr)__builtin_amdgcn_kernarg_segment_ptr();
+    asm volatile("" : "+s"(p));
+    return p;
+}
+
+template <typename SymT>
+__device__ __forceinline__ void finish_sub(uint32_t offA, uint32_t offB, uint32_t L, uint32_t fatal, uint32_t Kp, double S,
+                                           uint32_t skipped, uint32_t cm, bool packed, SubScore& out) {
+    if (packed) {
+        skipped >>= 2;
+        cm >>= 2;
+    }
+    const uint32_t cn = 16u * ((L + 15u) >> 4) - skipped;
+    const bool rescan = L != 0u && S != S;
+    const bool ok = L != 0u && cn != 0u && S < __builtin_inf();
+    const double* __restrict__ inv_n = coop_args_here()->st.inv_n;
+    const double x = inv_n[ok ? cn : 0u] * S;
+    out.x = ok ? x : -__builtin_inf();
+    out.mm = ok ? cm : 1u;
+    out.n = ok ? cn : 1u;
+    out.err = fatal;
+    if (__ballot(rescan) != 0ull) {
+        if (rescan) {
+            const char* sym = (const char*)coop_args_here()->st.sym;
+            const SubScore e = score_sub_slow<SymT>((const SymT*)(sym + offA), (const SymT*)(sym + offB), L, Kp);
+            out.x = e.x;
+            out.mm = e.mm;
+            out.n = e.n;
+            out.err |= e.err;
+        }
+    }
+}
+
+template <typename SymT, int LG, int DEPTH = 1>
+__device__ __forceinline__ void score_sub_coop(__amdgpu_buffer_rsrc_t rsrc, uint32_t oob, uint32_t stage, uint32_t offA, uint32_t offB, uint32_t L,
+                                               uint32_t fatal, uint32_t Kp, SubScore& out) {
+    using T = Tr<SymT>;
+    constexpr uint32_t kSymB = sizeof(SymT);
+    constexpr int kChunks = 4 / kSymB;
+    constexpr uint32_t kChunkB = 16u * kSymB;
+    constexpr bool kPacked = !(sizeof(SymT) == 1 && LG >= 6);
+    const uint32_t lane = threadIdx.x & 63u;
+    const uint32_t piece = (lane & 3u) ^ ((lane >> 4) & 3u);
+    const uint32_t Lb = L * kSymB;
+    uint32_t la[4], lb[4], lim[4];
+#pragma unroll
+    for (int j = 0; j < 4; ++j) {
+        const int src = 16 * j + (int)(lane >> 2);
+        la[j] = (uint32_t)__shfl((int)offA, src, 64) + 16u * piece;
+        lb[j] = (uint32_t)__shfl((int)offB, src, 64) + 16u * piece;
+        const uint32_t end = (uint32_t)__shfl((int)Lb, src, 64), cs = (16u * piece) & ~(kChunkB - 1u);
+        lim[j] = end > cs ? end - cs : 0u;
+    }
+    const uint32_t wr = stage + lane * 16u;
+    const uint32_t rd = stage + lane * 64u + (((lane >> 2) & 3u) << 4);
+    if constexpr (DEPTH == 0) {
+        double S = 0.0;
+        uint32_t skipped = 0, cm = 0;
+        const uint32_t rdA = stage + lane * 64u + (((lane >> 2) & 3u) << 4), rdB = rdA + 4096u;
+        auto fetch_dma = [&](uint32_t at) {
+#pragma unroll
+            for (int j = 0; j < 4; ++j) {
+                const bool on = at < lim[j];
+#if !(HC_ABLATE & 8)
+                __builtin_amdgcn_raw_ptr_buffer_load_lds(rsrc, (__attribute__((address_space(3))) void*)(uintptr_t)(stage + 1024u * j), 16,
+                                                         on ? la[j] : oob, at, 0, 0);
+#endif
+                __builtin_amdgcn_raw_ptr_buffer_load_lds(rsrc, (__attribute__((address_space(3))) void*)(uintptr_t)(stage + 4096u + 1024u * j), 16,
+                                                         on ? lb[j] : oob, at, 0, 0);
+            }
+        };
+#if HC_ABLATE & 16
+        if (__ballot(Lb != 0u) != 0ull) {
+            auto fetch_b = [&](uint32_t at, uint32_t half) {
+#pragma unroll
+                for (int j = 0; j < 4; ++j) {
+                    const bool on = at < lim[j];
+                    __builtin_amdgcn_raw_ptr_buffer_load_lds(rsrc, (__attribute__((address_space(3))) void*)(uintptr_t)(stage + 4096u * half + 1024u * j), 16,
+                                                             on ? lb[j] : oob, at, 0, 0);
+                }
+            };
+            fetch_b(0, 0);
+            fetch_b(64u, 1);
+            uint32_t half = 0;
+            for (uint32_t at = 0;; at += 64u, half ^= 1u) {
+                asm volatile("s_waitcnt vmcnt(4)" ::: "memory");
+                wave_lds_order();
+                u32x4 xa[4], xb[4];
+                const uint32_t rdH = rdA + 4096u * half;
+#pragma unroll
+                for (int p = 0; p < 4; ++p) {
+                    xb[p] = lds_load128(rdH ^ ((uint32_t)p << 4));
+                    xa[p] = xb[p];
+                }
+                asm volatile("s_waitcnt lgkmcnt(0)" : "+v"(xa[0]), "+v"(xa[1]), "+v"(xa[2]), "+v"(xa[3]), "+v"(xb[0]), "+v"(xb[1]), "+v"(xb[2]), "+v"(xb[3])::"memory");
+                wave_lds_order();
+                const bool more = __ballot(at + 64u < Lb) != 0ull;
+                fetch_b(at + 128u, half);
+                uint32_t cn4 = 0, cm4 = 0;
+#pragma unroll
+                for (int q = 0; q < kChunks; ++q)
+                    if (at + kChunkB * q < Lb) {
+                        uint32_t wa[T::kWords], wb[T::kWords];
+#pragma unroll
+                        for (int sw = 0; sw < (int)kSymB; ++sw) {
+                            const int p = q * (int)kSymB + sw;
+#pragma unroll
+                            for (int w = 0; w < 4; ++w) {
+                                wa[4 * sw + w] = xa[p][w] ^ 0x08080808u;
+                                wb[4 * sw + w] = xb[p][w];
+                            }
+                        }
+#pragma unroll
+                        for (int h = 0; h < 2; ++h) {
+                            double t[8];
+                            half_chunk_terms<SymT, LG>(wa + h * (T::kWords / 2), wb + h * (T::kWords / 2), Kp, t, cn4, cm4);
+#pragma unroll
+                            for (int k = 0; k < 8; ++k) S += t[k];
+                        }
+                    }
+                skipped = __builtin_amdgcn_sad_u8(cn4, 0u, skipped);
+                cm = __builtin_amdgcn_sad_u8(cm4, 0u, cm);
+                if (!more) break;
+            }
+            asm volatile("s_waitcnt vmcnt(0)" ::: "memory");
+        }
+        finish_sub<SymT>(offA, offB, L, fatal, Kp, S == S ? S : 0.0, skipped, cm, kPacked, out);
+        return;
+#endif
+        if (__ballot(Lb != 0u) != 0ull) {
+            fetch_dma(0);
+            for (uint32_t at = 0;; at += 64u) {
+                asm volatile("s_waitcnt vmcnt(0)" ::: "memory");
+                wave_lds_order();
+                u32x4 xa[4], xb[4];
+#pragma unroll
+                for (int p = 0; p < 4; ++p) {
+                    xb[p] = lds_load128(rdB ^ ((uint32_t)p << 4));
+#if HC_ABLATE & 8
+                    xa[p] = xb[p] ^ 0x08080808u;
+#else
+                    xa[p] = lds_load128(rdA ^ ((uint32_t)p << 4));
+#endif
+                }
+                asm volatile("s_waitcnt lgkmcnt(0)" : "+v"(xa[0]), "+v"(xa[1]), "+v"(xa[2]), "+v"(xa[3]), "+v"(xb[0]), "+v"(xb[1]), "+v"(xb[2]), "+v"(xb[3])::"memory");
+                wave_lds_order();
+                const bool more = __ballot(at + 64u < Lb) != 0ull;
+                if (more) fetch_dma(at + 64u);
+                uint32_t cn4 = 0, cm4 = 0;
+#pragma unroll
+                for (int q = 0; q < kChunks; ++q)
+                    if (at + kChunkB * q < Lb) {
+                        uint32_t wa[T::kWords], wb[T::kWords];
+#pragma unroll
+                        for (int sw = 0; sw < (int)kSymB; ++sw) {
+                            const int p = q * (int)kSymB + sw;
+#pragma unroll
+                            for (int w = 0; w < 4; ++w) {
+                                wa[4 * sw + w] = xa[p][w];
+                                wb[4 * sw + w] = xb[p][w];
+                            }
+                        }
+#pragma unroll
+                        for (int h = 0; h < 2; ++h) {
+                            double t[8];
+                            half_chunk_terms<SymT, LG>(wa + h * (T::kWords / 2), wb + h * (T::kWords / 2), Kp, t, cn4, cm4);
+#pragma unroll
+                            for (int k = 0; k < 8; ++k) S += t[k];
+                        }
+                    }
+                if (kPacked) {
+                    skipped = __builtin_amdgcn_sad_u8(cn4, 0u, skipped);
+                    cm = __builtin_amdgcn_sad_u8(cm4, 0u, cm);
+                } else {
+                    skipped += cn4;
+                    cm += cm4;
+                }
+                if (!more) break;
+            }
+        }
+        finish_sub<SymT>(offA, offB, L, fatal, Kp, S, skipped, cm, kPacked, out);
+        return;
+    }
+    u32x4 nA[DEPTH == 0 ? 1 : DEPTH][4], nB[DEPTH == 0 ? 1 : DEPTH][4];
+    auto fetch = [&](u32x4 (&sA)[4], u32x4 (&sB)[4], uint32_t at) {
+#pragma unroll
+        for (int j = 0; j < 4; ++j) {
+            const bool on = at < lim[j];
+#if HC_ABLATE & 2
+            sA[j] = u32x4{0x01010101u + (on ? (la[j] + at) & 0x02020202u : 0u), 0x01010101u, 0x09090909u, 0x11111111u};
+            sB[j] = u32x4{0x09090909u + (on ? (lb[j] + at) & 0x02020202u : 0u), 0x09090909u, 0x01010101u, 0x11111111u};
+#else
+            sA[j] = __builtin_amdgcn_raw_buffer_load_b128(rsrc, on ? la[j] : oob, at, 0);
+            sB[j] = __builtin_amdgcn_raw_buffer_load_b128(rsrc, on ? lb[j] : oob, at, 0);
+#endif
+        }
+    };
+    double S = 0.0;
+    uint32_t skipped = 0, cm = 0;
+    auto step = [&](u32x4 (&sA)[4], u32x4 (&sB)[4], uint32_t at) {
+        u32x4 xa[4];
+#if HC_ABLATE & 4
+        u32x4 xb_[4];
+#pragma unroll
+        for (int p = 0; p < 4; ++p) {
+            xa[p] = sA[p];
+            xb_[p] = sB[p];
+        }
+#else
+#pragma unroll
+        for (int j = 0; j < 4; ++j) lds_store128(wr + 1024u * j, sA[j]);
+        wave_lds_order();
+#pragma unroll
+        for (int p = 0; p < 4; ++p) xa[p] = lds_load128(rd ^ ((uint32_t)p << 4));
+        wave_lds_order();
+#pragma unroll
+        for (int j = 0; j < 4; ++j) lds_store128(wr + 1024u * j, sB[j]);
+        wave_lds_order();
+#endif
+        fetch(sA, sB, at + 64u * DEPTH);
+        uint32_t cn4 = 0, cm4 = 0;
+#pragma unroll
+        for (int q = 0; q < kChunks; ++q)
+            if (at + kChunkB * q < Lb) {
+                uint32_t wa[T::kWords], wb[T::kWords];
+#pragma unroll
+                for (int s = 0; s < (int)kSymB; ++s) {
+                    const int p = q * (int)kSymB + s;
+#if HC_ABLATE & 4
+                    const u32x4 vb = xb_[p];
+#else
+                    const u32x4 vb = lds_load128(rd ^ ((uint32_t)p << 4));
+#endif
+#pragma unroll
+                    for (int w = 0; w < 4; ++w) {
+                        wa[4 * s + w] = xa[p][w];
+                        wb[4 * s + w] = vb[w];
+                    }
+                }
+#pragma unroll
+                for (int h = 0; h < 2; ++h) {
+                    double t[8];
+                    half_chunk_terms<SymT, LG>(wa + h * (T::kWords / 2), wb + h * (T::kWords / 2), Kp, t, cn4, cm4);
+#pragma unroll
+                    for (int k = 0; k < 8; ++k) S += t[k];
+                }
+            }
+        if (kPacked) {
+            skipped = __builtin_amdgcn_sad_u8(cn4, 0u, skipped);
+            cm = __builtin_amdgcn_sad_u8(cm4, 0u, cm);
+        } else {
+            skipped += cn4;
+            cm += cm4;
+        }
+        wave_lds_order();
+    };
+#pragma unroll
+    for (int d = 0; d < DEPTH; ++d) fetch(nA[d], nB[d], 64u * d);
+    for (uint32_t at = 0; __ballot(at < Lb) != 0ull; at += 64u * DEPTH) {
+        step(nA[0], nB[0], at);
+        if (DEPTH == 2) {
+            if (__ballot(at + 64u < Lb) == 0ull) break;
+            step(nA[DEPTH - 1], nB[DEPTH - 1], at + 64u);
+        }
+    }
+    finish_sub<SymT>(offA, offB, L, fatal, Kp, S, skipped, cm, kPacked, out);
+}
+
+template <bool STREAM = true>
+__device__ __forceinline__ void store_result(hc_result_rec* __restrict__ out, uint64_t i, const hc_result_rec& r) {
+    unsigned long long* p = (unsigned long long*)(out + i);
+    if (STREAM) {
+        __builtin_nontemporal_store((unsigned long long)__double_as_longlong(r.x1), p);
+        __builtin_nontemporal_store((unsigned long long)__double_as_longlong(r.x2), p + 1);
+        __builtin_nontemporal_store(((unsigned long long)r.n_cls << 32) | r.mm, p + 2);
+    } else {
+        p[0] = (unsigned long long)__double_as_longlong(r.x1);
+        p[1] = (unsigned long long)__double_as_longlong(r.x2);
+        p[2] = ((unsigned long long)r.n_cls << 32) | r.mm;
+    }
+}
+
+__device__ __forceinline__ uint32_t band_test(double x, const Band& b) { return x > b.hi ? 1u : (x <= b.lo ? 0u : 2u); }
+
+struct ClassParams {
+    Band edge, ov;
+    double merge_contigs;
+    uint32_t flags;
+};
+__device__ __forceinline__ ClassParams class_params(const ScoreParams& prm) { return ClassParams{prm.edge, prm.ov, prm.merge_contigs, prm.flags}; }
+
+__device__ __forceinline__ uint32_t taken_here(uint32_t v) {
+    asm volatile("" : "+v"(v));
+    return v;
+}
+
+template <bool STREAM = true>
+__device__ __forceinline__ hc_result_rec classify_and_store(const ClassParams& prm, int ns, const SubScore& s1, const SubScore& s2,
+                                                            uint64_t i, hc_result_rec* __restrict__ out) {
+    hc_result_rec res;
+    const bool two = ns == 2;
+    bool second = two && (uint64_t)s1.mm * s2.n < (uint64_t)s2.mm * s1.n;
+    const bool large = two && !((s1.mm | s2.mm) < (1u << 24) && (s1.n | s2.n) < (1u << 26));
+    if (__ballot(large) != 0ull) {
+        const uint32_t m1 = taken_here(s1.mm);
+        if (large) second = (double)(float)m1 / (double)s1.n < (double)(float)s2.mm / (double)s2.n;
+    }
+    const uint32_t mm = second ? s2.mm : s1.mm, nn = second ? s2.n : s1.n;
+    const bool e_all = prm.flags & 1u, o_all = prm.flags & 2u;
+    uint32_t e = e_all ? 1u : band_test(s1.x, prm.edge);
+    uint32_t o = o_all ? 1u : band_test(s1.x, prm.ov);
+    {
+        const uint32_t e2 = (e_all || !two) ? 1u : band_test(s2.x, prm.edge), o2 = (o_all || !two) ? 1u : band_test(s2.x, prm.ov);
+        e = (e == 0 || e2 == 0) ? 0u : ((e == 1 && e2 == 1) ? 1u : 2u);
+        o = (o == 0 || o2 == 0) ? 0u : ((o == 1 && o2 == 1) ? 1u : 2u);
+    }
+    bool mc = mm == 0u;
+    if (prm.merge_contigs != 0.0) mc = (double)(float)taken_here(mm) / (double)nn <= prm.merge_contigs;
+    uint32_t cls = o == 1 ? HC_CLS_NONEDGE : (o == 2 ? HC_CLS_AMBIG : HC_CLS_DROP);
+    cls = mc ? HC_CLS_EDGE_MC : cls;
+    cls = e == 1 ? HC_CLS_EDGE : (e == 2 ? HC_CLS_AMBIG : cls);
+    cls = (s1.err | s2.err) ? HC_CLS_ERROR : cls;
+    cls = ns <= 0 ? (ns == 0 ? HC_CLS_ERROR : HC_CLS_DROP) : cls;
+    res.x1 = s1.x;
+    res.x2 = s2.x;
+    res.mm = mm;
+    res.n_cls = (nn & 0x0FFFFFFFu) | (cls << 28);
+    store_result<STREAM>(out, i, res);
+    return res;
+}
+
+template <typename SymT, int G, int LG>
+__device__ __forceinline__ hc_result_rec score_candidate(const ScoreParams& prm, const SymT* __restrict__ sym, uint32_t Kp, int ns,
+                                                         const Sub& sub0, const Sub& sub1, uint64_t i,
+                                                         hc_result_rec* __restrict__ out) {
+    if (ns <= 0) {
+        hc_result_rec res;
+        res.x1 = -__builtin_inf();
+        res.x2 = __builtin_nan("");
+        res.mm = 1;
+        res.n_cls = 1u | ((ns == 0 ? HC_CLS_ERROR : HC_CLS_DROP) << 28);
+        store_result(out, i, res);
+        return res;
+    }
+    SubScore s1, s2;
+    s2.x = __builtin_nan("");
+    s2.mm = 0;
+    s2.n = 1;
+    s2.err = 0;
+    const SymT* a1 = sym + sub1.offA + sub1.pos;
+    const SymT* b1 = sym + sub1.offB;
+    const uint32_t L1 = ns == 2 ? sub_positions(sub1, prm.min_read_len) | (sub1.fatal << 31) : 0u;
+    score_sub_wide<SymT, LG, G>(sym + sub0.offA + sub0.pos, sym + sub0.offB, sub_positions(sub0, prm.min_read_len), sub0.fatal, Kp, s1);
+    if (ns == 2) score_sub_wide<SymT, LG, G>(a1, b1, L1 & 0x7FFFFFFFu, L1 >> 31, Kp, s2);
+    return classify_and_store(class_params(prm), ns, s1, s2, i, out);
+}
 
 __device__ __forceinline__ void append_rows_block(const RowSink& sink, bool valid, const hc_result_rec& res, uint64_t i, uint32_t* lds4) {
     const bool keep = valid && (res.n_cls >> 28) != HC_CLS_DROP;
@@ -1069,10 +1096,14 @@
 }
 
 template <typename SymT, int LG, int WG, bool SORT, bool DYN, int DEPTH = 1, bool WQ = false>
-__global__ __launch_bounds__(WG, DEPTH == 2 ? 2 : (WG == 256 ? 4 : (WG == 512 ? 2 : 1))) void score_kernel_coop(StoreView st, ScoreParams prm, const double* __restrict__ lut_g,
-                                                            const void* __restrict__ in, uint64_t n, hc_result_rec* __restrict__ out,
-                                                            const uint32_t* __restrict__ perm, RowSink sink, uint32_t* __restrict__ queue) {
+__global__ __launch_bounds__(WG, DEPTH == 2 ? 2 : (WG == 256 ? 4 : (WG == 512 ? 2 : 1))) void score_kernel_coop(CoopArgs args) {
     static_assert(SORT && (WQ || !DYN), "score_kernel_coop: no launch takes the unsorted form or the bucketed form without tickets");
+    const StoreView& st = args.st;
+    const ScoreParams& prm = args.prm;
+    const double* __restrict__ lut_g = args.lut_g;
+    const void* __restrict__ in = args.in;
+    uint64_t n = args.n;
+    const uint32_t* __restrict__ perm = args.perm;
     const uint64_t n_hint = n;
     if (prm.n_dev) {
         const uint64_t nd = *prm.n_dev;
@@ -1089,15 +1120,13 @@
     if (threadIdx.x == 0) {
         scratch[24] = 0;
         scratch[29] = 0;
-        if (sink.started) atomicAdd(sink.started, 1ull);
+        if (args.sink.started) atomicAdd(args.sink.started, 1ull);
     }
     __syncthreads();
     const uint32_t stage_base = coop_stage_base(st.lut_bytes, WG);
     const uint32_t stage = (uint32_t)__builtin_amdgcn_readfirstlane(
         (int)(stage_base + (threadIdx.x >> 6) * (DEPTH == 0 ? 2u * kStageBytesPerWave : kStageBytesPerWave)));
-    const SymT* sym = (const SymT*)st.sym;
     const uint32_t Kp = st.K + 2u;
-    const uint32_t fmt = prm.rec_fmt;
     const __amdgpu_buffer_rsrc_t rsrc = __builtin_amdgcn_make_buffer_rsrc((void*)st.sym, 0, (uint32_t)st.store_bytes, 0x00020000);
     const uint32_t oob = (uint32_t)st.store_bytes;
     const uint32_t tid = threadIdx.x;
@@ -1161,22 +1190,28 @@
         int ns = -2;
         uint32_t a0 = 0, b0 = 0, l0 = 0, a1 = 0, b1 = 0, l1 = 0;
         if (slot < n) {
+            const coop_args_ptr ks = coop_args_here();
             i = perm ? (uint64_t)perm[slot] : slot;
-            const Cand rec = load_cand(in, i, fmt);
-            if (st.regular) {
-                ns = resolve_regular32<(int)sizeof(SymT)>(st, prm.min_read_len, rec, a0, b0, l0, a1, b1, l1);
+            const Cand rec = load_cand(ks->in, i, ks->prm.rec_fmt);
+            if (ks->st.regular) {
+                const RegularGeom g{ks->st.n_reads, ks->st.n_single, ks->st.seq_syms, ks->st.ulen, ks->prm.min_read_len};
+                ns = resolve_regular32<(int)sizeof(SymT)>(g, rec, a0, b0, l0, a1, b1, l1);
             } else {
                 Sub sub0{}, sub1{};
-                ns = resolve<(int)sizeof(SymT)>(st, rec, sub0, sub1);
+                StoreView sv{};
+                sv.reads = ks->st.reads;
+                sv.n_reads = ks->st.n_reads;
+                const uint32_t min_read_len = ks->prm.min_read_len;
+                ns = resolve<(int)sizeof(SymT)>(sv, rec, sub0, sub1);
                 if (ns >= 1) {
                     a0 = (uint32_t)((sub0.offA + sub0.pos) * sizeof(SymT));
                     b0 = (uint32_t)(sub0.offB * sizeof(SymT));
-                    l0 = sub_positions(sub0, prm.min_read_len) | (sub0.fatal << 31);
+                    l0 = sub_positions(sub0, min_read_len) | (sub0.fatal << 31);
                 }
                 if (ns == 2) {
                     a1 = (uint32_t)((sub1.offA + sub1.pos) * sizeof(SymT));
                     b1 = (uint32_t)(sub1.offB * sizeof(SymT));
-                    l1 = sub_positions(sub1, prm.min_read_len) | (sub1.fatal << 31);
+                    l1 = sub_positions(sub1, min_read_len) | (sub1.fatal << 31);
                 }
             }
         }
@@ -1216,13 +1251,13 @@
             const u32x4 p0 = lds_load128(x + 16u * lane), p1 = lds_load128(x + 16u * (127u - lane));
             wave_lds_order();
             SubScore r[2];
-            score_sub_coop<SymT, LG, DEPTH>(rsrc, oob, sym, stage, p0[0], p0[1], p0[2] & 0x7FFFFFFFu, p0[2] >> 31, Kp, st.inv_n, r[0]);
+            score_sub_coop<SymT, LG, DEPTH>(rsrc, oob, stage, p0[0], p0[1], p0[2] & 0x7FFFFFFFu, p0[2] >> 31, Kp, r[0]);
             r[1].x = -__builtin_inf();
             r[1].mm = 1;
             r[1].n = 1;
             r[1].err = p1[2] >> 31;
             if (__ballot((p1[2] & 0x7FFFFFFFu) != 0u) != 0ull)
-                score_sub_coop<SymT, LG, DEPTH>(rsrc, oob, sym, stage, p1[0], p1[1], p1[2] & 0x7FFFFFFFu, p1[2] >> 31, Kp, st.inv_n, r[1]);
+                score_sub_coop<SymT, LG, DEPTH>(rsrc, oob, stage, p1[0], p1[1], p1[2] & 0x7FFFFFFFu, p1[2] >> 31, Kp, r[1]);
             wave_lds_order();
             lds_store128(x + 16u * p0[3], u32x4{(uint32_t)__double2loint(r[0].x), (uint32_t)__double2hiint(r[0].x), r[0].mm, r[0].n | (r[0].err << 31)});
             lds_store128(x + 16u * p1[3], u32x4{(uint32_t)__double2loint(r[1].x), (uint32_t)__double2hiint(r[1].x), r[1].mm, r[1].n | (r[1].err << 31)});
@@ -1244,28 +1279,26 @@
             s2.n = 1;
             s2.err = 0;
         }
+        const coop_args_ptr ka = coop_args_here();
         hc_result_rec res;
         res.n_cls = 0;
         if (slot < n) {
-            if (ns <= 0) {
-                res.x1 = -__builtin_inf();
-                res.x2 = __builtin_nan("");
-                res.mm = 1;
-                res.n_cls = 1u | ((ns == 0 ? HC_CLS_ERROR : HC_CLS_DROP) << 28);
-                store_result<!DYN>(out, i, res);
-            } else {
-                res = classify_and_store<!DYN>(prm, ns, s1, s2, i, out);
-            }
-        }
-        if (sink.rows) {
+            const ClassParams cp{Band{ka->prm.edge.lo, ka->prm.edge.hi}, Band{ka->prm.ov.lo, ka->prm.ov.hi}, ka->prm.merge_contigs, ka->prm.flags};
+            res = classify_and_store<!DYN>(cp, ns, s1, s2, i, ka->out);
+        }
+        if (ka->sink.rows) {
+            const RowSink sink{ka->sink.rows,      ka->sink.count,     ka->sink.cap,      ka->sink.base_index, ka->sink.lines_in,
+                               ka->sink.lines_out, ka->sink.seg_buf,   ka->sink.seg_count, ka->sink.seg_rows,  ka->sink.spill_cap,
+                               ka->sink.spill_buf, ka->sink.spill_count, ka->sink.started};
             if (sink.seg_count) append_rows_segment(sink, slot < n, res, i, seg_counter);
             else if (DYN) append_rows_wave(sink, slot < n, res, i);
             else append_rows_block(sink, slot < n, res, i, scratch);
         }
     }
-    if (sink.rows && sink.seg_count) {
+    const coop_args_ptr ke = coop_args_here();
+    if (ke->sink.rows && ke->sink.seg_count) {
         __syncthreads();
-        if (threadIdx.x == 0) sink.seg_count[blockIdx.x] = scratch[24];
+        if (threadIdx.x == 0) ke->sink.seg_count[blockIdx.x] = scratch[24];
     }
 }
 
@@ -1448,8 +1481,10 @@
     }
     if (k.wq) prm.pad = (prm.pad & 0xFFu) | (kTicketSteps << 8);
     uint32_t* queue = plan.bucketed ? b.bucket_queue : nullptr;
-    void* args[] = {(void*)&st, &prm, &lut_g, &in, &n, &out, &perm, &sink, &queue};
-    const hipError_t le = hipLaunchKernel(k.fn, dim3(plan.blocks), dim3(k.wg), args, plan.lds, stream);
+    CoopArgs coop{st, prm, lut_g, in, n, out, perm, sink, queue};
+    void* coop_args[] = {&coop};
+    void* lane_args[] = {(void*)&st, &prm, &lut_g, &in, &n, &out, &perm, &sink};
+    const hipError_t le = hipLaunchKernel(k.fn, dim3(plan.blocks), dim3(k.wg), k.coop ? coop_args : lane_args, plan.lds, stream);
     if (plan.segmented) {
         hipLaunchKernelGGL(sink_compact_kernel, dim3(plan.blocks), dim3(256), 0, stream, (const hc_gather_row*)b.seg_buf, (const uint32_t*)b.seg_count,
                            sink.seg_rows, plan.blocks, b.rows, (unsigned long long)b.cap, b.row_count, (const hc_gather_row*)sink.spill_buf,
diff --git a/haploconduct_amd/csrc/hc_resolve.h b/haploconduct_amd/csrc/hc_resolve.h
--- a/haploconduct_amd/csrc/hc_resolve.h
+++ b/haploconduct_amd/csrc/hc_resolve.h
@@ -128,45 +128,31 @@
     return 2;
 }
 
+struct RegularGeom {
+    uint32_t n_reads, n_single, seq_syms, ulen, min_read_len;
+};
 template <int SB>
-__device__ __forceinline__ int resolve_regular32(const StoreView& st, uint32_t min_read_len, const Cand& r, uint32_t& a0, uint32_t& b0, uint32_t& L0,
-                                                 uint32_t& a1, uint32_t& b1, uint32_t& L1) {
-    a0 = b0 = L0 = a1 = b1 = L1 = 0u;
-    if (r.skip) return -1;
-    if (r.read1 >= st.n_reads || r.read2 >= st.n_reads || r.read1 == r.read2) return 0;
+__device__ __forceinline__ int resolve_regular32(const RegularGeom& st, const Cand& r, uint32_t& a0, uint32_t& b0, uint32_t& L0, uint32_t& a1,
+                                                 uint32_t& b1, uint32_t& L1) {
     const uint32_t slot = st.seq_syms >> 1;
     const bool p1 = r.read1 >= st.n_single, p2 = r.read2 >= st.n_single;
+    const bool bad = r.read1 >= st.n_reads || r.read2 >= st.n_reads || r.read1 == r.read2 || (p1 && p2 && r.ord != '1' && r.ord != '2');
+    const int ns = r.skip ? -1 : (bad ? 0 : ((p1 || p2) ? 2 : 1));
     const uint32_t base1 = (p1 ? 2u * r.read1 - st.n_single : r.read1) * st.seq_syms;
     const uint32_t base2 = (p2 ? 2u * r.read2 - st.n_single : r.read2) * st.seq_syms;
     const uint32_t F1 = base1 + (r.ori1 ? 0u : (p1 ? 3u * slot : slot));
     const uint32_t F2 = base2 + (r.ori2 ? 0u : (p2 ? 3u * slot : slot));
-    const uint32_t ok = st.ulen >= min_read_len ? st.ulen : 0u;
+    const uint32_t ok = st.ulen >= st.min_read_len ? st.ulen : 0u;
     a0 = (F1 + r.pos1) * SB;
     b0 = F2 * SB;
-    L0 = r.pos1 < ok ? ok - r.pos1 : 0u;
-    if (!p1 && !p2) return 1;
+    L0 = (ns >= 1 && r.pos1 < ok) ? ok - r.pos1 : 0u;
     const uint32_t K1 = p1 ? base1 + (r.ori1 ? slot : 2u * slot) : F1;
     const uint32_t K2 = p2 ? base2 + (r.ori2 ? slot : 2u * slot) : F2;
-    uint32_t A, B;
-    if (!p1) {
-        A = F1;
-        B = K2;
-    } else if (!p2) {
-        A = F2;
-        B = K1;
-    } else if (r.ord == '1') {
-        A = K1;
-        B = K2;
-    } else if (r.ord == '2') {
-        A = K2;
-        B = K1;
-    } else {
-        return 0;
-    }
-    a1 = (A + r.pos2) * SB;
-    b1 = B * SB;
-    L1 = r.pos2 < ok ? ok - r.pos2 : 0u;
-    return 2;
+    const bool swap = p1 && (!p2 || r.ord == '2');
+    a1 = ((swap ? K2 : K1) + r.pos2) * SB;
+    b1 = (swap ? K1 : K2) * SB;
+    L1 = (ns == 2 && r.pos2 < ok) ? ok - r.pos2 : 0u;
+    return ns;
 }
 
 __device__ __forceinline__ uint32_t sub_positions(const Sub& s, uint32_t min_read_len) {
```

After: 17.61 billion candidate overlaps/s (median of 6 runs). 1.02x the previous value.
